# Geo3DSmart/PDANet

Measured on AMD Instinct MI355X. Metric: scenes/sec (16384-pt ONCE, PDA-SSD forward+backward), higher is better.
Workload: dtype f32; 1 GPU; once16k_b2_detector_fwd_bwd_adam; scenes_per_gpu=2, global_batch=2, parallelism=dp1, world_size_seen=1, cpu_affinity=GPU-local NUMA node of 0000:5d:00.0: 128 CPUs, full=False, graph_tail=False, graph_head=True

## Files before the change

### include/pda_train.h

```cpp
#ifndef PDA_TRAIN_H
#define PDA_TRAIN_H
#include "pda_pointnet2.h"

#ifdef __cplusplus
extern "C" {
#endif

int pda_grad_norm(const float *g, int64_t n, float *norm_out, float *scratch1024, pda_stream_t stream);
int pda_adam_onecycle_step(float *p, const float *g, float *m, float *v, int64_t n, float lr,
                           float beta1, float beta2, float eps, float wd, int step,
                           const float *total_norm, float max_norm, pda_stream_t stream);

int64_t pda_bn_relu_scratch_bytes(int c);
int pda_bn_relu_fwd(const float *x, const float *gamma, const float *beta, float *running_mean,
                    float *running_var, float *y, float *mean_invstd, void *scratch, int64_t rows, int c,
                    float eps, float momentum, pda_stream_t stream);
int pda_bn_relu_bwd(const float *x, const float *grad_y, const float *gamma, const float *beta,
                    const float *mean_invstd, float *grad_x, float *grad_gamma, float *grad_beta,
                    void *scratch, int64_t rows, int c, pda_stream_t stream);
int pda_bn_relu_fwd_counted(const float *x, const float *gamma, const float *beta, float *running_mean, float *running_var,
                            float *y, float *mean_invstd, void *scratch, int64_t rows, int c, float eps, float momentum,
                            const int32_t *count, int32_t *status, int relu, int training, pda_stream_t stream);
int pda_bn_relu_bwd_counted(const float *x, const float *grad_y, const float *gamma, const float *beta,
                            const float *mean_invstd, float *grad_x, float *grad_gamma, float *grad_beta, void *scratch,
                            int64_t rows, int c, const int32_t *count, int relu, int training, pda_stream_t stream);
int pda_bn_relu_bwd_reduce(const float *x, const float *grad_y, const float *gamma, const float *beta,
                           const float *mean_invstd, float *grad_gamma, float *grad_beta, float *sums, void *scratch,
                           int64_t rows, int c, pda_stream_t stream);
int pda_bn_relu_fwd_mixed(const void *x, int x_is_bf16, const float *gamma, const float *beta, float *running_mean,
                          float *running_var, void *y, int y_is_bf16, float *mean_invstd, void *scratch,
                          int64_t rows, int c, float eps, float momentum, pda_stream_t stream);
int pda_bn_relu_bwd_mixed(const void *x, int x_is_bf16, const void *grad_y, int grad_y_is_bf16, const float *gamma,
                          const float *beta, const float *mean_invstd, void *grad_x, float *grad_gamma,
                          float *grad_beta, void *scratch, int64_t rows, int c, pda_stream_t stream);
int pda_bn_relu_max_pool_fwd(const void *x, int x_is_bf16, const float *gamma, const float *beta, float *running_mean,
                             float *running_var, float *out, uint8_t *arg, float *mean_invstd, void *scratch,
                             int64_t groups, int ns, int c, float eps, float momentum, pda_stream_t stream);
int pda_bn_relu_max_pool_bwd(const void *x, int x_is_bf16, const float *grad_out, const uint8_t *arg,
                             const float *gamma, const float *beta, const float *mean_invstd, void *grad_x,
                             float *grad_gamma, float *grad_beta, void *scratch, int64_t groups, int ns, int c,
                             pda_stream_t stream);

int64_t pda_layer_norm_scratch_bytes(int d);
int pda_layer_norm_fwd(const float *x, const float *residual, const float *gamma, const float *beta,
                       float *sum_out, float *y, float *mean_rstd, int64_t rows, int d, float eps,
                       pda_stream_t stream);
int pda_layer_norm_bwd(const float *x, const float *grad_y, const float *grad_y2, const float *gamma,
                       const float *mean_rstd, float *grad_x, float *grad_gamma, float *grad_beta,
                       void *scratch, int64_t rows, int d, pda_stream_t stream);
int pda_layer_norm_fwd_mixed(const void *x, int x_is_bf16, const float *residual, const float *gamma,
                             const float *beta, float *sum_out, float *y, uint16_t *y_bf16, float *mean_rstd,
                             int64_t rows, int d, float eps, pda_stream_t stream);
int pda_layer_norm_bwd_mixed(const float *x, const float *grad_y, const void *grad_y2, int grad_y2_is_bf16,
                             const float *gamma, const float *mean_rstd, float *grad_x, uint16_t *grad_x_bf16,
                             float *grad_gamma, float *grad_beta, void *scratch, int64_t rows, int d,
                             pda_stream_t stream);

int64_t pda_linear_wgrad_scratch_bytes(int64_t tokens, int in_features, int out_features);
int pda_linear_wgrad_form(int64_t tokens, int in_features, int out_features);
int pda_linear_wgrad(const float *x, const float *grad_out, float *grad_weight, float *grad_bias,
                     void *scratch, int64_t tokens, int in_features, int out_features, pda_stream_t stream);
int pda_linear_wgrad_bn(const float *x, const float *grad_out, float *grad_weight, float *grad_bias, void *scratch,
                        int64_t tokens, int in_features, int out_features, const float *x_mean_invstd,
                        const float *x_gamma, const float *x_beta, pda_stream_t stream);

int64_t pda_gemm_split_bn_tiles(int64_t tokens);
int pda_gemm_split_bn(const float *x, const void *wf, float *y, int64_t tokens, int k, int n_out,
                      const float *in_mean_invstd, const float *in_gamma, const float *in_beta, int stats_mode,
                      double *partial, pda_stream_t stream);
int pda_gemm_split_maxpool(const float *x, const void *wf, const float *bias, float *out, int64_t tokens, int k, int n_out,
                           int ns, int relu, pda_stream_t stream);
int pda_gemm_split_gather(const float *point_rows, const float *xyz, const float *new_xyz, const int32_t *idx,
                          const float *w1, int ldw1, const float *bias1, const void *wf, const float *bias2, float *y,
                          int b, int n, int m, int ns, int k, int n_out, int relu, pda_stream_t stream);
int pda_bn_stats_fwd(const float *x, float *running_mean, float *running_var, float *mean_invstd, void *scratch,
                     int64_t rows, int c, float eps, float momentum, pda_stream_t stream);
int pda_bn_finalize_fwd(const double *partial, int nblocks, int c, int64_t count, float eps, float momentum,
                        float *mean_invstd, float *running_mean, float *running_var, pda_stream_t stream);
int pda_bn_relu_max_pool_apply(const float *x, const float *gamma, const float *beta, const float *mean_invstd,
                               float *out, uint8_t *arg, int64_t groups, int ns, int c, pda_stream_t stream);

int64_t pda_colsum_scratch_bytes(int cols);
int pda_colsum_bf16(const uint16_t *g, float *out, void *scratch, int64_t rows, int cols, pda_stream_t stream);

int pda_assemble_tokens(const float *rppe, const float *dscale, const float *feats, const int32_t *idx,
                        const float *glob, float *out, int b, int n, int m, int nsample, int c,
                        pda_stream_t stream);
int pda_assemble_tokens_grad(const float *grad_out, const float *dscale, const float *feats, const int32_t *idx,
                             float *grad_rppe, float *grad_dscale, float *grad_feats, float *grad_glob,
                             int b, int n, int m, int nsample, int c, pda_stream_t stream);

int pda_add_max_pool(const float *a, const float *b, float *out, uint8_t *arg, int64_t groups, int seq, int d,
                     pda_stream_t stream);
int pda_max_pool_scatter(const float *grad_out, const uint8_t *arg, float *grad_x, int64_t groups, int seq,
                         int d, pda_stream_t stream);
int pda_add_max_pool_bf16(const float *a, const uint16_t *b, float *out, uint8_t *arg, int64_t groups, int seq,
                          int d, pda_stream_t stream);
int pda_max_pool_scatter_bf16(const float *grad_out, const uint8_t *arg, float *grad_x, uint16_t *grad_x_bf16,
                              int64_t groups, int seq, int d, pda_stream_t stream);

int pda_bn_relu_fwd_weighted(const float *x, const float *gamma, const float *beta, float *running_mean,
                             float *running_var, float *y, float *mean_invstd, void *scratch, int64_t rows, int c,
                             float eps, float momentum, const float *row_weight, int64_t count, pda_stream_t stream);
int pda_bn_relu_bwd_weighted(const float *x, const float *grad_y, const float *gamma, const float *beta,
                             const float *mean_invstd, float *grad_x, float *grad_gamma, float *grad_beta,
                             void *scratch, int64_t rows, int c, const float *row_weight, int64_t count,
                             pda_stream_t stream);

int pda_ragged_plan(const int32_t *idx, int32_t *cnt, int32_t *off, int32_t *rowmap, float *row_weight, int64_t groups,
                    int nsample, pda_stream_t stream);
int pda_assemble_tokens_ragged(const float *rppe, const float *dscale, const float *feats, const int32_t *idx,
                               const float *glob, const int32_t *rowmap, const int32_t *off, float *out,
                               int64_t max_tokens, int b, int n, int m, int nsample, int c, int rppe_compact,
                               pda_stream_t stream);
int pda_assemble_tokens_ragged_grad(const float *grad_out, const float *dscale, const float *feats,
                                    const int32_t *idx, const int32_t *cnt, const int32_t *off, const int32_t *rowmap,
                                    float *grad_rppe, float *grad_dscale, float *grad_feats, float *grad_glob,
                                    int64_t max_tokens, int b, int n, int m, int nsample, int c, int rppe_compact,
                                    pda_stream_t stream);
int pda_add_max_pool_ragged(const float *a, const float *b, const int32_t *cnt, const int32_t *off, float *out,
                            uint8_t *arg, int64_t groups, int d, pda_stream_t stream);
int pda_max_pool_scatter_ragged(const float *grad_out, const uint8_t *arg, const int32_t *rowmap,
                                const int32_t *off, float *grad_x, int64_t max_tokens, int64_t groups, int nsample,
                                int d, pda_stream_t stream);
int pda_group_attention_ragged_fwd(const float *qkv, const int32_t *cnt, const int32_t *off, float *out, float *lse,
                                   int64_t tokens, int64_t num_groups, int seq, int heads, int head_dim,
                                   pda_stream_t stream);
int pda_group_attention_ragged_bwd(const float *qkv, const float *grad_out, const float *lse, const int32_t *cnt,
                                   const int32_t *off, float *grad_qkv, int64_t tokens, int64_t num_groups, int seq,
                                   int heads, int head_dim, pda_stream_t stream);

int pda_densitynet_param_count(void);
int64_t pda_densitynet_scratch_bytes(void);
int pda_densitynet_fwd(const float *x, const float *params, float *y, float *stats, void *scratch,
                       float *running_mean1, float *running_var1, float *running_mean2, float *running_var2,
                       float *running_mean3, float *running_var3, int64_t n, float eps, float momentum,
                       pda_stream_t stream);
int pda_densitynet_bwd(const float *x, const float *grad_y, const float *params, const float *stats,
                       float *grad_params, void *scratch, int64_t n, float eps, pda_stream_t stream);
int pda_densitynet_fwd_unique(const float *x, const float *params, float *y, float *stats, void *scratch,
                              float *running_mean1, float *running_var1, float *running_mean2, float *running_var2,
                              float *running_mean3, float *running_var3, int64_t n, const int32_t *rowmap,
                              const float *row_weight, const int32_t *n_unique, int nsample, float eps, float momentum,
                              pda_stream_t stream);
int pda_densitynet_bwd_unique(const float *x, const float *grad_y, const float *params, const float *stats,
                              float *grad_params, void *scratch, int64_t n, const int32_t *rowmap,
                              const float *row_weight, const int32_t *n_unique, int nsample, float eps,
// ... 390 lines not shown
```

### pdanet_amd/_lib.py

```python
import ctypes
import os

_HERE = os.path.dirname(os.path.abspath(__file__))
LIB_PATH = os.environ.get("PDA_LIB_PATH") or os.path.join(_HERE, "libpda_pointnet2.so")
ABI_VERSION = 20


class DensityNetScale(ctypes.Structure):
    _fields_ = [("x", ctypes.c_void_p), ("grad_y", ctypes.c_void_p), ("params", ctypes.c_void_p), ("y", ctypes.c_void_p),
                ("stats", ctypes.c_void_p), ("scratch", ctypes.c_void_p), ("running", ctypes.c_void_p * 6),
                ("grad_params", ctypes.c_void_p), ("n", ctypes.c_int64), ("rowmap", ctypes.c_void_p),
                ("row_weight", ctypes.c_void_p), ("n_unique", ctypes.c_void_p), ("nsample", ctypes.c_int),
                ("eps", ctypes.c_float), ("momentum", ctypes.c_float)]


class OnceFrames(ctypes.Structure):
    _fields_ = [("gt_boxes", ctypes.c_void_p), ("gt_name", ctypes.c_void_p), ("gt_offsets", ctypes.c_void_p),
                ("pred_boxes", ctypes.c_void_p), ("pred_score", ctypes.c_void_p), ("pred_name", ctypes.c_void_p),
                ("pred_start", ctypes.c_void_p), ("pred_count", ctypes.c_void_p), ("iou_start", ctypes.c_void_p),
                ("n_gt_total", ctypes.c_int64), ("pred_cap", ctypes.c_int64), ("iou_cap", ctypes.c_int64),
                ("n_frames", ctypes.c_int), ("max_gt", ctypes.c_int), ("max_pred", ctypes.c_int)]


class KittiFrames(ctypes.Structure):
    _fields_ = [(n, ctypes.c_void_p) for n in ("gt_bbox", "gt_loc", "gt_dims", "gt_ry", "gt_alpha", "gt_trunc", "gt_occ",
                                               "gt_name", "gt_offsets", "dt_bbox", "dt_box", "dt_alpha", "dt_score",
                                               "dt_name", "dt_start", "dt_count", "ov_start", "frame_mode")] + \
               [("n_gt_total", ctypes.c_int64), ("det_cap", ctypes.c_int64), ("ov_cap", ctypes.c_int64),
                ("n_frames", ctypes.c_int), ("max_gt", ctypes.c_int), ("max_det", ctypes.c_int)]


PARAM_EPOCH = [0]
WEIGHT_EPOCH = [0]

_vp = ctypes.c_void_p
_i = ctypes.c_int
_f = ctypes.c_float

SIGNATURES = {
    "pda_furthest_point_sampling": [_vp, _vp, _vp, _i, _i, _i, _vp],
    "pda_furthest_point_sampling_with_dist": [_vp, _vp, _vp, _i, _i, _i, _vp],
    "pda_gather_points": [_vp, _vp, _vp, _i, _i, _i, _i, _vp],
    "pda_gather_points_grad": [_vp, _vp, _vp, _i, _i, _i, _i, _vp],
    "pda_ball_query": [_vp, _vp, _vp, _i, _i, _i, _f, _i, _vp],
    "pda_ball_query_dilated": [_vp, _vp, _vp, _i, _i, _i, _f, _f, _i, _vp],
    "pda_ellipsoid_query": [_vp, _vp, _vp, _i, _i, _i, _f, _f, _f, _i, _vp],
    "pda_ball_query_cells_scratch_bytes": [_i, _i],
    "pda_ball_query_cells": [_vp, _vp, ctypes.POINTER(_vp), _i, _i, _i, _i, ctypes.POINTER(_f), ctypes.POINTER(ctypes.c_int32),
                             _vp, ctypes.c_int64, _vp],
    "pda_ball_query_multi": [_vp, _vp, ctypes.POINTER(_vp), _i, _i, _i, _i,
                             ctypes.POINTER(_f), ctypes.POINTER(ctypes.c_int32), _vp],
    "pda_group_points": [_vp, _vp, _vp, _i, _i, _i, _i, _i, _vp],
    "pda_group_points_grad": [_vp, _vp, _vp, _i, _i, _i, _i, _i, _vp],
    "pda_group_rows": [_vp, _vp, _vp, _i, _i, _i, ctypes.c_int64, _vp],
    "pda_group_rows_grad": [_vp, _vp, _vp, _i, _i, _i, ctypes.c_int64, _vp],
    "pda_three_nn": [_vp, _vp, _vp, _vp, _i, _i, _i, _vp],
    "pda_three_interpolate": [_vp, _vp, _vp, _vp, _i, _i, _i, _i, _vp],
    "pda_three_interpolate_grad": [_vp, _vp, _vp, _vp, _i, _i, _i, _i, _vp],
    "pda_chamfer_forward": [_vp, _vp, _vp, _vp, _vp, _vp, _i, _i, _i, _vp],
    "pda_chamfer_backward": [_vp, _vp, _vp, _vp, _vp, _vp, _vp, _vp, _i, _i, _i, _vp],
    "pda_group_attention_fwd": [_vp, _vp, _vp, ctypes.c_int64, _i, _i, _i, _vp],
    "pda_group_attention_bwd": [_vp, _vp, _vp, _vp, ctypes.c_int64, _i, _i, _i, _vp],
    "pda_group_attention_fwd_bf16": [_vp, _vp, _vp, ctypes.c_int64, _i, _i, _i, _vp],
    "pda_group_attention_bwd_bf16": [_vp, _vp, _vp, _vp, ctypes.c_int64, _i, _i, _i, _vp],
    "pda_sa_mlp_maxpool": [_vp, _vp, _vp, _vp, _vp, _i, _i, _i, _i, _i, ctypes.POINTER(ctypes.c_int32),
                           ctypes.POINTER(_vp), ctypes.POINTER(_vp), ctypes.POINTER(_vp), _vp],
    "pda_linear_cols_packed_size": [_i, _i],
    "pda_linear_cols_pack": [_vp, _vp, _i, _i, _i, _i, _vp],
    "pda_linear_cols": [_vp, _vp, _vp, ctypes.c_int64, _i, _i, _vp],
    "pda_sa_gather_linear": [_vp, _vp, _vp, _vp, _vp, _vp, _i, _i, _i, _i, _i, _i, _vp],
    "pda_linear_split_packed_bytes": [_i, _i],
    "pda_linear_split_pack": [_vp, _vp, _i, _i, _i, _vp],
    "pda_linear_split_pack_both": [_vp, _vp, _vp, _i, _i, _vp],
    "pda_linear_split": [_vp, _vp, _vp, _vp, ctypes.c_int64, _i, _i, _i, _vp],
    "pda_gemm_split": [_vp, _vp, _vp, _vp, ctypes.c_int64, _i, _i, _i, _i, _vp],
    "pda_sa_mlp_packed_size": [_i, _i, _i],
    "pda_sa_mlp_pack_weights": [_vp, _vp, _i, _i, _i, _vp],
    "pda_grad_norm": [_vp, ctypes.c_int64, _vp, _vp, _vp],
    "pda_bn_relu_scratch_bytes": [_i],
    "pda_bn_relu_fwd": [_vp, _vp, _vp, _vp, _vp, _vp, _vp, _vp, ctypes.c_int64, _i, _f, _f, _vp],
    "pda_bn_relu_bwd": [_vp, _vp, _vp, _vp, _vp, _vp, _vp, _vp, _vp, ctypes.c_int64, _i, _vp],    "pda_bn_relu_fwd_mixed": [_vp, _i, _vp, _vp, _vp, _vp, _vp, _i, _vp, _vp, ctypes.c_int64, _i, _f, _f, _vp],
    "pda_bn_relu_bwd_mixed": [_vp, _i, _vp, _i, _vp, _vp, _vp, _vp, _vp, _vp, _vp, ctypes.c_int64, _i, _vp],
    "pda_bn_relu_max_pool_fwd": [_vp, _i, _vp, _vp, _vp, _vp, _vp, _vp, _vp, _vp, ctypes.c_int64, _i, _i, _f, _f, _vp],
    "pda_bn_relu_max_pool_bwd": [_vp, _i, _vp, _vp, _vp, _vp, _vp, _vp, _vp, _vp, _vp, ctypes.c_int64, _i, _i, _vp],

    "pda_layer_norm_scratch_bytes": [_i],
    "pda_layer_norm_fwd": [_vp, _vp, _vp, _vp, _vp, _vp, _vp, ctypes.c_int64, _i, _f, _vp],
    "pda_layer_norm_bwd": [_vp, _vp, _vp, _vp, _vp, _vp, _vp, _vp, _vp, ctypes.c_int64, _i, _vp],
    "pda_layer_norm_fwd_mixed": [_vp, _i, _vp, _vp, _vp, _vp, _vp, _vp, _vp, ctypes.c_int64, _i, _f, _vp],
    "pda_layer_norm_bwd_mixed": [_vp, _vp, _vp, _i, _vp, _vp, _vp, _vp, _vp, _vp, _vp, ctypes.c_int64, _i, _vp],
    "pda_linear_wgrad_scratch_bytes": [ctypes.c_int64, _i, _i],
    "pda_linear_wgrad_form": [ctypes.c_int64, _i, _i],
    "pda_linear_wgrad": [_vp, _vp, _vp, _vp, _vp, ctypes.c_int64, _i, _i, _vp],
    "pda_linear_wgrad_bn": [_vp, _vp, _vp, _vp, _vp, ctypes.c_int64, _i, _i, _vp, _vp, _vp, _vp],
    "pda_gemm_split_bn_tiles": [ctypes.c_int64],
    "pda_gemm_split_bn": [_vp, _vp, _vp, ctypes.c_int64, _i, _i, _vp, _vp, _vp, _i, _vp, _vp],
    "pda_gemm_split_maxpool": [_vp, _vp, _vp, _vp, ctypes.c_int64, _i, _i, _i, _i, _vp],
    "pda_gemm_split_gather": [_vp, _vp, _vp, _vp, _vp, _i, _vp, _vp, _vp, _vp, _i, _i, _i, _i, _i, _i, _i, _vp],
    "pda_bn_stats_fwd": [_vp, _vp, _vp, _vp, _vp, ctypes.c_int64, _i, _f, _f, _vp],
    "pda_bn_finalize_fwd": [_vp, _i, _i, ctypes.c_int64, _f, _f, _vp, _vp, _vp, _vp],
    "pda_bn_relu_max_pool_apply": [_vp, _vp, _vp, _vp, _vp, _vp, ctypes.c_int64, _i, _i, _vp],
    "pda_bn_relu_bwd_reduce": [_vp, _vp, _vp, _vp, _vp, _vp, _vp, _vp, _vp, ctypes.c_int64, _i, _vp],
    "pda_colsum_scratch_bytes": [_i],
    "pda_colsum_bf16": [_vp, _vp, _vp, ctypes.c_int64, _i, _vp],
    "pda_assemble_tokens": [_vp, _vp, _vp, _vp, _vp, _vp, _i, _i, _i, _i, _i, _vp],
    "pda_assemble_tokens_grad": [_vp, _vp, _vp, _vp, _vp, _vp, _vp, _vp, _i, _i, _i, _i, _i, _vp],
    "pda_add_max_pool": [_vp, _vp, _vp, _vp, ctypes.c_int64, _i, _i, _vp],
    "pda_max_pool_scatter": [_vp, _vp, _vp, ctypes.c_int64, _i, _i, _vp],
    "pda_add_max_pool_bf16": [_vp, _vp, _vp, _vp, ctypes.c_int64, _i, _i, _vp],
    "pda_max_pool_scatter_bf16": [_vp, _vp, _vp, _vp, ctypes.c_int64, _i, _i, _vp],
    "pda_ragged_plan": [_vp, _vp, _vp, _vp, _vp, ctypes.c_int64, _i, _vp],
    "pda_assemble_tokens_ragged": [_vp, _vp, _vp, _vp, _vp, _vp, _vp, _vp, ctypes.c_int64, _i, _i, _i, _i, _i, _i, _vp],
    "pda_assemble_tokens_ragged_grad": [_vp, _vp, _vp, _vp, _vp, _vp, _vp, _vp, _vp, _vp, _vp, ctypes.c_int64, _i, _i, _i, _i, _i, _i, _vp],
    "pda_bn_relu_fwd_weighted": [_vp, _vp, _vp, _vp, _vp, _vp, _vp, _vp, ctypes.c_int64, _i, _f, _f, _vp, ctypes.c_int64, _vp],
    "pda_bn_relu_bwd_weighted": [_vp, _vp, _vp, _vp, _vp, _vp, _vp, _vp, _vp, ctypes.c_int64, _i, _vp, ctypes.c_int64, _vp],
    "pda_add_max_pool_ragged": [_vp, _vp, _vp, _vp, _vp, _vp, ctypes.c_int64, _i, _vp],
    "pda_max_pool_scatter_ragged": [_vp, _vp, _vp, _vp, _vp, ctypes.c_int64, ctypes.c_int64, _i, _i, _vp],
    "pda_group_attention_ragged_fwd": [_vp, _vp, _vp, _vp, _vp, ctypes.c_int64, ctypes.c_int64, _i, _i, _i, _vp],
    "pda_group_attention_ragged_bwd": [_vp, _vp, _vp, _vp, _vp, _vp, ctypes.c_int64, ctypes.c_int64, _i, _i, _i, _vp],
    "pda_densitynet_param_count": [],
    "pda_densitynet_eval_param_count": [],
    "pda_densitynet_scratch_bytes": [],
    "pda_densitynet_fwd": [_vp, _vp, _vp, _vp, _vp, _vp, _vp, _vp, _vp, _vp, _vp, ctypes.c_int64, _f, _f, _vp],
    "pda_densitynet_bwd": [_vp, _vp, _vp, _vp, _vp, _vp, ctypes.c_int64, _f, _vp],
    "pda_densitynet_eval": [_vp, _vp, _vp, ctypes.c_int64, _vp],
    "pda_densitynet_fwd_multi": [_vp, _i, _vp],
    "pda_densitynet_bwd_multi": [_vp, _i, _vp],
    "pda_densitynet_fwd_unique": [_vp, _vp, _vp, _vp, _vp, _vp, _vp, _vp, _vp, _vp, _vp, ctypes.c_int64, _vp, _vp, _vp, _i, _f, _f, _vp],
    "pda_densitynet_bwd_unique": [_vp, _vp, _vp, _vp, _vp, _vp, ctypes.c_int64, _vp, _vp, _vp, _i, _f, _vp],
    "pda_pda_geometry": [_vp, _vp, _vp, _vp, _vp, _i, _i, _i, _i, _f, _vp],
    "pda_points_in_boxes": [_vp, _vp, _vp, _i, _i, _i, _vp],
    "pda_roiaware_pool3d_fwd": [_vp, _vp, _vp, _vp, _vp, _vp, _i, _i, _i, _i, _i, _i, _i, _i, _vp],
    "pda_roiaware_pool3d_bwd": [_vp, _vp, _vp, _vp, _i, _i, _i, _i, _i, _i, _i, _i, _vp],
    "pda_roipoint_pool3d_fwd": [_vp, _vp, _vp, _vp, _vp, _i, _i, _i, _i, _i, _vp],
    "pda_points_in_boxes_mask": [_vp, _vp, _vp, _i, _i, _vp],
    "pda_points_in_boxes_count": [_vp, _i, _vp, _vp, _i, _i, _i, _vp],
    "pda_assign_point_targets": [_vp, _vp, _vp, _vp, _vp, _vp, _i, _i, _i, _i, _i, _vp],
    "pda_sa_gaussian_mask": [_vp, _i, _i, _vp, _vp, _vp, ctypes.c_int64, _vp],
    "pda_head_assign_targets": [_vp, _i, _i, _vp, ctypes.POINTER(ctypes.c_float), _vp, _vp, _vp, _vp, _vp, _i, _i, _i, _i, _i, _i, _vp],
    "pda_head_cls_loss": [_vp, _i, _i, _i, _vp, _vp, ctypes.c_int64, _f, _vp, _vp, _vp],
    "pda_head_centerness": [_vp, _vp, _vp, _vp, ctypes.c_int64, _vp],
    "pda_head_box_loss": [_vp, _vp, _vp, _vp, _f, _i, _f, _f, ctypes.c_int64, _vp, _vp, _vp],
    "pda_head_vote_loss": [_i, _vp, _vp, _vp, _vp, _i, _i, _i, _f, ctypes.c_int64, _vp, _vp, _vp],
    "pda_head_corner_loss": [_vp, _vp, _vp, _i, _vp, _vp, _vp, _i, _f, ctypes.c_int64, _vp, _vp, _vp, _vp],
    "pda_boxes_overlap_bev": [_vp, _vp, _vp, _i, _i, _vp],
    "pda_boxes_iou_bev": [_vp, _vp, _vp, _i, _i, _vp],
    "pda_nms_mask_words": [_i],
    "pda_nms_bev": [_vp, _vp, _vp, _vp, _vp, _i, _i, _f, _i, _vp],
    "pda_sa_small_train_workspace_bytes": [],
    "pda_sa_small_train_supported": [_i, _i, _i, _i, _i, ctypes.c_int64],
    "pda_sa_small_train_fwd": [_vp] * 7 + [ctypes.POINTER(_vp)] * 4 + [ctypes.POINTER(_f)] * 2 + [_vp] * 4 + [_i] * 8 + [_vp],
    "pda_sa_small_train_bwd": [_vp] * 13 + [ctypes.POINTER(_vp)] * 2 + [_i] * 8 + [_vp],
    "pda_sa_xyz_grad_scratch_bytes": [_i],
    "pda_sa_point_gather": [_vp, _vp, _vp, _vp, _vp, _i, _vp, _i, _vp, _i, _i, _i, _i, _i, _vp],
    "pda_sa_xyz_grad": [_vp, _vp, _vp, _vp, _vp, _i, _vp, _i, _vp, _vp, _i, _i, _i, _i, _i, _vp],
    "pda_sa_point_gather_stats_blocks": [ctypes.c_int64, _i],
    "pda_sa_point_gather_stats": [_vp, _vp, _vp, _vp, _vp, _i, _vp, _vp, _i, _i, _i, _i, _i, _vp],
    "pda_sa_point_grad_bn": [_vp] * 10 + [_i, _vp, _i, _vp, _vp, _vp, _i, _i, _i, _i, _i, _vp],
    "pda_adam_onecycle_step": [_vp, _vp, _vp, _vp, ctypes.c_int64, _f, _f, _f, _f, _f, _i, _vp, _f, _vp],
    "pda_input_stage_workspace_bytes": [_i, ctypes.c_int64],
    "pda_input_stage": [_vp, _vp, ctypes.c_int64, _i, _i, ctypes.c_int64, ctypes.POINTER(_f), _i, _vp, _vp, _vp,
                        ctypes.c_uint64, _i, _vp, _vp, _vp, _vp],
    "pda_input_boxes": [_vp, _vp, ctypes.c_int64, _i, _i, _i, ctypes.POINTER(_f), _i, _vp, _vp, _vp],
    "pda_augment_workspace_bytes": [_i, ctypes.c_int64, _i],
    "pda_augment": [_vp, _vp, ctypes.c_int64, _i, _i, ctypes.c_int64, _vp, _vp, ctypes.c_int64, _vp, _vp, ctypes.c_int64, _vp,
                    _vp, _vp, _i, _vp, _vp, _vp, _i, _vp, _vp, _vp, ctypes.POINTER(_f), ctypes.c_int64, _vp, ctypes.c_int64,
                    _vp, _vp, ctypes.c_int64, _vp, _vp, _vp, _vp],
    "pda_augment_paste": [_vp, _vp, ctypes.c_int64, _i, _i, ctypes.c_int64, _vp, _vp, ctypes.c_int64, _vp, _vp, ctypes.c_int64, _vp,
                          _vp, _vp, _i, _vp, _vp, _vp, _i, ctypes.POINTER(_f), ctypes.c_int64, _vp, ctypes.c_int64, _vp, _vp,
                          ctypes.c_int64, _vp, _vp, _vp, _vp],
    "pda_augment_steps_workspace_bytes": [_i, ctypes.c_int64, _i, _i],
    "pda_augment_steps": [_vp, _vp, ctypes.c_int64, _i, _i, ctypes.c_int64, _vp, _vp, ctypes.c_int64,
                          ctypes.POINTER(ctypes.c_int32), _i, _vp, _vp, _i, _i, _vp, _vp, ctypes.c_int64, _vp, _vp,
                          ctypes.c_int64, _vp, _vp, _vp, _vp],
    "pda_pyramid_aug_workspace_bytes": [_i, ctypes.c_int64, _i],
    "pda_pyramid_aug": [_vp, _vp, ctypes.c_int64, _i, _i, ctypes.c_int64, _vp, _vp, ctypes.c_int64, _vp, _vp, _vp, _vp, _vp, _i,
                        ctypes.POINTER(ctypes.c_double), _i, _i, _i, _vp, _vp, ctypes.c_int64, _vp, _vp, ctypes.c_int64, _vp,
# ... 172 lines not shown
```

### pdanet_amd/csrc/layer_norm.hip

```cpp
#include "pda_common.h"

namespace pda {

constexpr int LN_BLOCKS = 1024;

__device__ __forceinline__ float wave_sum(float v) {
#pragma unroll
    for (int o = 32; o >= 1; o >>= 1) v += __shfl_xor(v, o);
    return v;
}

template <int V, bool RESIDUAL, typename TX>
__global__ __launch_bounds__(256) void layer_norm_fwd_kernel(const TX* __restrict__ x, const float* __restrict__ res,
                                                             const float* __restrict__ gamma, const float* __restrict__ beta,
                                                             float* __restrict__ sum_out, float* __restrict__ y,
                                                             bf16_t* __restrict__ yb, float* __restrict__ mean_rstd, int64_t rows,
                                                             float eps) {
    constexpr int D = 256 * V;
    const int lane = lane_id();
    float4 g[V], be[V];
#pragma unroll
    for (int v = 0; v < V; ++v) {
        g[v] = reinterpret_cast<const float4*>(gamma)[v * 64 + lane];
        be[v] = reinterpret_cast<const float4*>(beta)[v * 64 + lane];
    }
    for (int64_t r = (int64_t)blockIdx.x * 4 + wave_id(); r < rows; r += (int64_t)gridDim.x * 4) {
        float4 a[V];
        float s = 0.f;
#pragma unroll
        for (int v = 0; v < V; ++v) {
            a[v] = load4(x + r * D + 4 * (v * 64 + lane));
            if (RESIDUAL) {
                const float4 b = reinterpret_cast<const float4*>(res + r * D)[v * 64 + lane];
                a[v].x += b.x; a[v].y += b.y; a[v].z += b.z; a[v].w += b.w;
                reinterpret_cast<float4*>(sum_out + r * D)[v * 64 + lane] = a[v];
            }
            s += (a[v].x + a[v].y) + (a[v].z + a[v].w);
        }
        const float mean = wave_sum(s) * (1.0f / D);
        float q = 0.f;
#pragma unroll
        for (int v = 0; v < V; ++v) {
            const float dx = a[v].x - mean, dy = a[v].y - mean, dz = a[v].z - mean, dw = a[v].w - mean;
            q += (dx * dx + dy * dy) + (dz * dz + dw * dw);
        }
        const float rstd = 1.0f / sqrtf(wave_sum(q) * (1.0f / D) + eps);
#pragma unroll
        for (int v = 0; v < V; ++v) {
            float4 o;
            o.x = (a[v].x - mean) * rstd * g[v].x + be[v].x;
            o.y = (a[v].y - mean) * rstd * g[v].y + be[v].y;
            o.z = (a[v].z - mean) * rstd * g[v].z + be[v].z;
            o.w = (a[v].w - mean) * rstd * g[v].w + be[v].w;
            if (y) reinterpret_cast<float4*>(y + r * D)[v * 64 + lane] = o;
            if (yb) store4(yb + r * D + 4 * (v * 64 + lane), o);
        }
        if (lane == 0) { mean_rstd[r * 2] = mean; mean_rstd[r * 2 + 1] = rstd; }
    }
}

template <int V, bool TWO, typename T2>
__global__ __launch_bounds__(256) void layer_norm_bwd_kernel(const float* __restrict__ x, const float* __restrict__ dy,
                                                             const T2* __restrict__ dy2, const float* __restrict__ gamma,
                                                             const float* __restrict__ mean_rstd, float* __restrict__ dx,
                                                             bf16_t* __restrict__ dxb, float* __restrict__ partial, int64_t rows) {
    constexpr int D = 256 * V;
    __shared__ float red[2][4][D];
    const int lane = lane_id(), w = wave_id();
    float4 g[V], sb[V], sg[V];
#pragma unroll
    for (int v = 0; v < V; ++v) {
        g[v] = reinterpret_cast<const float4*>(gamma)[v * 64 + lane];
        sb[v] = make_float4(0, 0, 0, 0); sg[v] = make_float4(0, 0, 0, 0);
    }
    for (int64_t r = (int64_t)blockIdx.x * 4 + w; r < rows; r += (int64_t)gridDim.x * 4) {
        const float mean = mean_rstd[r * 2], rstd = mean_rstd[r * 2 + 1];
        float4 xh[V], d[V];
        float s1 = 0.f, s2 = 0.f;
#pragma unroll
        for (int v = 0; v < V; ++v) {
            const float4 xv = reinterpret_cast<const float4*>(x + r * D)[v * 64 + lane];
            d[v] = reinterpret_cast<const float4*>(dy + r * D)[v * 64 + lane];
            if (TWO) {
                const float4 e = load4(dy2 + r * D + 4 * (v * 64 + lane));
                d[v].x += e.x; d[v].y += e.y; d[v].z += e.z; d[v].w += e.w;
            }
            xh[v] = make_float4((xv.x - mean) * rstd, (xv.y - mean) * rstd, (xv.z - mean) * rstd, (xv.w - mean) * rstd);
            sb[v].x += d[v].x; sb[v].y += d[v].y; sb[v].z += d[v].z; sb[v].w += d[v].w;
            sg[v].x += d[v].x * xh[v].x; sg[v].y += d[v].y * xh[v].y; sg[v].z += d[v].z * xh[v].z; sg[v].w += d[v].w * xh[v].w;
            d[v].x *= g[v].x; d[v].y *= g[v].y; d[v].z *= g[v].z; d[v].w *= g[v].w;
            s1 += (d[v].x + d[v].y) + (d[v].z + d[v].w);
            s2 += (d[v].x * xh[v].x + d[v].y * xh[v].y) + (d[v].z * xh[v].z + d[v].w * xh[v].w);
        }
        const float m1 = wave_sum(s1) * (1.0f / D), m2 = wave_sum(s2) * (1.0f / D);
#pragma unroll
        for (int v = 0; v < V; ++v) {
            float4 o;
            o.x = rstd * (d[v].x - m1 - xh[v].x * m2);
            o.y = rstd * (d[v].y - m1 - xh[v].y * m2);
            o.z = rstd * (d[v].z - m1 - xh[v].z * m2);
            o.w = rstd * (d[v].w - m1 - xh[v].w * m2);
            reinterpret_cast<float4*>(dx + r * D)[v * 64 + lane] = o;
            if (dxb) store4(dxb + r * D + 4 * (v * 64 + lane), o);
        }
    }
#pragma unroll
    for (int v = 0; v < V; ++v) {
        reinterpret_cast<float4*>(red[0][w])[v * 64 + lane] = sb[v];
        reinterpret_cast<float4*>(red[1][w])[v * 64 + lane] = sg[v];
    }
    __syncthreads();
    for (int c = threadIdx.x; c < D; c += 256) {
        partial[((size_t)blockIdx.x * 2 + 0) * D + c] = (red[0][0][c] + red[0][1][c]) + (red[0][2][c] + red[0][3][c]);
        partial[((size_t)blockIdx.x * 2 + 1) * D + c] = (red[1][0][c] + red[1][1][c]) + (red[1][2][c] + red[1][3][c]);
    }
}

__global__ __launch_bounds__(1024) void layer_norm_finalize_kernel(const float* __restrict__ partial, int nblocks, int d,
                                                                   float* __restrict__ dgamma, float* __restrict__ dbeta) {
    __shared__ float red[2][16][64];
    const int cl = threadIdx.x & 63, part = threadIdx.x >> 6;
    const int c = blockIdx.x * 64 + cl;
    float a = 0.f, b = 0.f;
    if (c < d) {
        float va[8], vb[8];
        for (int k0 = part; k0 < nblocks; k0 += 16 * 8) {
#pragma unroll
            for (int u = 0; u < 8; ++u) {
                const int k = k0 + 16 * u;
                va[u] = k < nblocks ? partial[((size_t)k * 2 + 0) * d + c] : 0.f;
                vb[u] = k < nblocks ? partial[((size_t)k * 2 + 1) * d + c] : 0.f;
            }
#pragma unroll
            for (int u = 0; u < 8; ++u) { a += va[u]; b += vb[u]; }
        }
    }
    red[0][part][cl] = a; red[1][part][cl] = b;
    __syncthreads();
    if (part != 0 || c >= d) return;
    float s1 = 0.f, s2 = 0.f;
#pragma unroll
    for (int p = 0; p < 16; ++p) { s1 += red[0][p][cl]; s2 += red[1][p][cl]; }
    dbeta[c] = s1;
    dgamma[c] = s2;
}

static int ln_grid(int64_t rows) {
    const int64_t b = divup64(rows, 4);
    return (int)(b < LN_BLOCKS ? b : LN_BLOCKS);
}

}

PDA_API int64_t pda_layer_norm_scratch_bytes(int d) { return (int64_t)pda::LN_BLOCKS * 2 * (d > 0 ? d : 0) * (int64_t)sizeof(float); }

namespace pda {

template <typename TX>
static int launch_layer_norm_fwd(const TX* x, const float* residual, const float* gamma, const float* beta, float* sum_out, float* y,
                                 bf16_t* yb, float* mean_rstd, int64_t rows, int d, float eps, hipStream_t st, const char* what) {
    PDA_REQUIRE(rows >= 0, "%s: rows = %lld", what, (long long)rows);
    PDA_REQUIRE(d == 256 || d == 512 || d == 1024, "%s: D = %d (256, 512 or 1024)", what, d);
    if (rows == 0) return PDA_OK;
    PDA_REQUIRE(x && gamma && beta && (y || yb) && mean_rstd, "%s: null pointer", what);
    PDA_REQUIRE((residual == nullptr) == (sum_out == nullptr), "%s: residual and sum_out come together", what);
    PDA_REQUIRE((((uintptr_t)y | (uintptr_t)gamma | (uintptr_t)beta | (uintptr_t)residual | (uintptr_t)sum_out) & 15) == 0 &&
                    (((uintptr_t)x | (uintptr_t)yb) & (4 * sizeof(TX) - 1) & 15) == 0 && ((uintptr_t)yb & 7) == 0,
                "%s: pointers must be 16-byte aligned (8 for bf16 tensors)", what);
    const dim3 grid(ln_grid(rows)), block(256);
#define PDA_LN_FWD(V)                                                                                                          \
    if (residual) hipLaunchKernelGGL((layer_norm_fwd_kernel<V, true, TX>), grid, block, 0, st, x, residual, gamma, beta, sum_out, y, yb, mean_rstd, rows, eps); \
    else hipLaunchKernelGGL((layer_norm_fwd_kernel<V, false, TX>), grid, block, 0, st, x, residual, gamma, beta, sum_out, y, yb, mean_rstd, rows, eps)
    if (d == 256) { PDA_LN_FWD(1); } else if (d == 512) { PDA_LN_FWD(2); } else { PDA_LN_FWD(4); }
#undef PDA_LN_FWD
    return check_launch(what);
}

template <typename T2>
static int launch_layer_norm_bwd(const float* x, const float* grad_y, const T2* grad_y2, const float* gamma, const float* mean_rstd,
                                 float* grad_x, bf16_t* grad_x_b, float* grad_gamma, float* grad_beta, void* scratch, int64_t rows, int d,
                                 hipStream_t st, const char* what) {
    PDA_REQUIRE(rows >= 1, "%s: rows = %lld", what, (long long)rows);
    PDA_REQUIRE(d == 256 || d == 512 || d == 1024, "%s: D = %d (256, 512 or 1024)", what, d);
    PDA_REQUIRE(x && grad_y && gamma && mean_rstd && grad_x && grad_gamma && grad_beta && scratch, "%s: null pointer", what);
    PDA_REQUIRE((((uintptr_t)x | (uintptr_t)grad_y | (uintptr_t)grad_x | (uintptr_t)gamma) & 15) == 0 &&
                    ((uintptr_t)grad_y2 & (4 * sizeof(T2) - 1)) == 0 && ((uintptr_t)grad_x_b & 7) == 0,
                "%s: pointers must be 16-byte aligned (8 for bf16 tensors)", what);
    const int nblocks = ln_grid(rows);
    const dim3 grid(nblocks), block(256);
    float* partial = (float*)scratch;
#define PDA_LN_BWD(V)                                                                                                               \
    if (grad_y2) hipLaunchKernelGGL((layer_norm_bwd_kernel<V, true, T2>), grid, block, 0, st, x, grad_y, grad_y2, gamma, mean_rstd, grad_x, grad_x_b, partial, rows); \
    else hipLaunchKernelGGL((layer_norm_bwd_kernel<V, false, T2>), grid, block, 0, st, x, grad_y, grad_y2, gamma, mean_rstd, grad_x, grad_x_b, partial, rows)
    if (d == 256) { PDA_LN_BWD(1); } else if (d == 512) { PDA_LN_BWD(2); } else { PDA_LN_BWD(4); }
#undef PDA_LN_BWD
    hipLaunchKernelGGL(layer_norm_finalize_kernel, dim3(divup(d, 64)), dim3(1024), 0, st, partial, nblocks, d, grad_gamma, grad_beta);
    return check_launch(what);
}

}

PDA_API int pda_layer_norm_fwd(const float* x, const float* residual, const float* gamma, const float* beta, float* sum_out,
                               float* y, float* mean_rstd, int64_t rows, int d, float eps, pda_stream_t stream) {
    PDA_REQUIRE(y != nullptr || rows == 0, "pda_layer_norm_fwd: null pointer");
    return pda::launch_layer_norm_fwd<float>(x, residual, gamma, beta, sum_out, y, nullptr, mean_rstd, rows, d, eps, (hipStream_t)stream,
                                             "pda_layer_norm_fwd");
}

PDA_API int pda_layer_norm_fwd_mixed(const void* x, int x_is_bf16, const float* residual, const float* gamma, const float* beta,
                                     float* sum_out, float* y, uint16_t* y_bf16, float* mean_rstd, int64_t rows, int d, float eps,
                                     pda_stream_t stream) {
    if (x_is_bf16)
        return pda::launch_layer_norm_fwd<pda::bf16_t>((const pda::bf16_t*)x, residual, gamma, beta, sum_out, y, y_bf16, mean_rstd, rows, d,
                                                       eps, (hipStream_t)stream, "pda_layer_norm_fwd_mixed");
    return pda::launch_layer_norm_fwd<float>((const float*)x, residual, gamma, beta, sum_out, y, y_bf16, mean_rstd, rows, d, eps,
                                             (hipStream_t)stream, "pda_layer_norm_fwd_mixed");
}

PDA_API int pda_layer_norm_bwd(const float* x, const float* grad_y, const float* grad_y2, const float* gamma, const float* mean_rstd,
                               float* grad_x, float* grad_gamma, float* grad_beta, void* scratch, int64_t rows, int d,
                               pda_stream_t stream) {
    return pda::launch_layer_norm_bwd<float>(x, grad_y, grad_y2, gamma, mean_rstd, grad_x, nullptr, grad_gamma, grad_beta, scratch, rows, d,
                                             (hipStream_t)stream, "pda_layer_norm_bwd");
}

PDA_API int pda_layer_norm_bwd_mixed(const float* x, const float* grad_y, const void* grad_y2, int grad_y2_is_bf16, const float* gamma,
                                     const float* mean_rstd, float* grad_x, uint16_t* grad_x_bf16, float* grad_gamma, float* grad_beta,
                                     void* scratch, int64_t rows, int d, pda_stream_t stream) {
    if (grad_y2_is_bf16)
        return pda::launch_layer_norm_bwd<pda::bf16_t>(x, grad_y, (const pda::bf16_t*)grad_y2, gamma, mean_rstd, grad_x, grad_x_bf16,
                                                       grad_gamma, grad_beta, scratch, rows, d, (hipStream_t)stream, "pda_layer_norm_bwd_mixed");
    return pda::launch_layer_norm_bwd<float>(x, grad_y, (const float*)grad_y2, gamma, mean_rstd, grad_x, grad_x_bf16, grad_gamma, grad_beta,
                                             scratch, rows, d, (hipStream_t)stream, "pda_layer_norm_bwd_mixed");
}

namespace pda {

template <typename TB>
__global__ __launch_bounds__(256) void add_max_pool_kernel(const float* __restrict__ a, const TB* __restrict__ b,
                                                           float* __restrict__ out, uint8_t* __restrict__ arg, int64_t groups,
                                                           int s, int d4) {
    const int64_t e = (int64_t)blockIdx.x * 256 + threadIdx.x;
    if (e >= groups * d4) return;
    const int64_t g = e / d4;
    const int c = (int)(e % d4);
    const float4* pa = reinterpret_cast<const float4*>(a) + (size_t)g * s * d4 + c;
    const TB* pb = b + 4 * ((size_t)g * s * d4 + c);
    float4 best = make_float4(-__builtin_inff(), -__builtin_inff(), -__builtin_inff(), -__builtin_inff());
    uchar4 bi = make_uchar4(0, 0, 0, 0);
    for (int t = 0; t < s; ++t) {
        const float4 x = pa[(size_t)t * d4], y = load4(pb + 4 * (size_t)t * d4);
        const float4 v = make_float4(x.x + y.x, x.y + y.y, x.z + y.z, x.w + y.w);
        if (v.x > best.x) { best.x = v.x; bi.x = (uint8_t)t; }
        if (v.y > best.y) { best.y = v.y; bi.y = (uint8_t)t; }
        if (v.z > best.z) { best.z = v.z; bi.z = (uint8_t)t; }
        if (v.w > best.w) { best.w = v.w; bi.w = (uint8_t)t; }
    }
    reinterpret_cast<float4*>(out)[e] = best;
    reinterpret_cast<uchar4*>(arg)[e] = bi;
}

__global__ __launch_bounds__(256) void max_pool_scatter_kernel(const float* __restrict__ dout, const uint8_t* __restrict__ arg,
                                                               float* __restrict__ dx, bf16_t* __restrict__ dxb, int64_t groups, int s,
                                                               int d4) {
    const int64_t e = (int64_t)blockIdx.x * 256 + threadIdx.x;
    if (e >= groups * s * d4) return;
    const int c = (int)(e % d4);
    const int t = (int)((e / d4) % s);
    const int64_t g = e / ((int64_t)d4 * s);
    const float4 v = reinterpret_cast<const float4*>(dout)[g * d4 + c];
    const uchar4 k = reinterpret_cast<const uchar4*>(arg)[g * d4 + c];
    const float4 o = make_float4(k.x == t ? v.x : 0.f, k.y == t ? v.y : 0.f, k.z == t ? v.z : 0.f, k.w == t ? v.w : 0.f);
    reinterpret_cast<float4*>(dx)[e] = o;
    if (dxb) store4(dxb + 4 * e, o);
}

}

namespace pda {

template <typename TB>
static int launch_add_max_pool(const float* a, const TB* b, float* out, uint8_t* arg, int64_t groups, int seq, int d, hipStream_t st,
                               const char* what) {
    PDA_REQUIRE(groups >= 0 && seq >= 1 && seq <= 255 && d >= 4 && (d & 3) == 0, "%s: groups=%lld seq=%d d=%d", what, (long long)groups, seq, d);
    if (groups == 0) return PDA_OK;
    PDA_REQUIRE(a && b && out && arg, "%s: null pointer", what);
    PDA_REQUIRE((((uintptr_t)a | (uintptr_t)out) & 15) == 0 && ((uintptr_t)b & (4 * sizeof(TB) - 1)) == 0 && ((uintptr_t)arg & 3) == 0,
                "%s: alignment", what);
    const int64_t n = groups * (d / 4);
    hipLaunchKernelGGL(add_max_pool_kernel<TB>, dim3((unsigned)divup64(n, 256)), dim3(256), 0, st, a, b, out, arg, groups, seq, d / 4);
    return check_launch(what);
}

static int launch_max_pool_scatter(const float* grad_out, const uint8_t* arg, float* grad_x, bf16_t* grad_x_b, int64_t groups, int seq, int d,
                                   hipStream_t st, const char* what) {
    PDA_REQUIRE(groups >= 0 && seq >= 1 && seq <= 255 && d >= 4 && (d & 3) == 0, "%s: groups=%lld seq=%d d=%d", what, (long long)groups, seq, d);
    if (groups == 0) return PDA_OK;
    PDA_REQUIRE(grad_out && arg && grad_x, "%s: null pointer", what);
    PDA_REQUIRE((((uintptr_t)grad_out | (uintptr_t)grad_x) & 15) == 0 && ((uintptr_t)arg & 3) == 0 && ((uintptr_t)grad_x_b & 7) == 0,
                "%s: alignment", what);
    const int64_t n = groups * seq * (d / 4);
    hipLaunchKernelGGL(max_pool_scatter_kernel, dim3((unsigned)divup64(n, 256)), dim3(256), 0, st, grad_out, arg, grad_x, grad_x_b, groups,
                       seq, d / 4);
    return check_launch(what);
}

}

PDA_API int pda_add_max_pool(const float* a, const float* b, float* out, uint8_t* arg, int64_t groups, int seq, int d,
                             pda_stream_t stream) {
    return pda::launch_add_max_pool<float>(a, b, out, arg, groups, seq, d, (hipStream_t)stream, "pda_add_max_pool");
}

PDA_API int pda_add_max_pool_bf16(const float* a, const uint16_t* b, float* out, uint8_t* arg, int64_t groups, int seq, int d,
                                  pda_stream_t stream) {
    return pda::launch_add_max_pool<pda::bf16_t>(a, b, out, arg, groups, seq, d, (hipStream_t)stream, "pda_add_max_pool_bf16");
// ... 13 lines not shown
```

### pdanet_amd/csrc/wgrad.hip

```cpp
#include "pda_common.h"
#include "split_bf16.h"

#include <stdlib.h>

namespace pda {

typedef float f32x16 __attribute__((ext_vector_type(16)));

constexpr int WG_KC = 32;
constexpr int WG_TILE = 128;

__device__ __forceinline__ void lds_dma16(const float* gsrc, float* lds_dst_wave_uniform) {
    uint32_t keep;
    const uint32_t dst = __builtin_amdgcn_readfirstlane((uint32_t)(uintptr_t)lds_dst_wave_uniform);
    asm volatile("s_mov_b32 %0, m0\n\ts_mov_b32 m0, %2\n\ts_nop 0\n\tglobal_load_lds_dwordx4 %1, off\n\ts_mov_b32 m0, %0"
                 : "=&s"(keep) : "v"(gsrc), "s"(dst) : "memory");
}

__global__ __launch_bounds__(256) void wgrad_kernel(const float* __restrict__ X, const float* __restrict__ G,
                                                    float* __restrict__ part_w, float* __restrict__ part_b, int64_t T, int M,
                                                    int N, int tiles_m, int tiles_n, int S, int64_t KS, int nblocks) {
    __shared__ __attribute__((aligned(16))) float ldsG[2][WG_KC][WG_TILE];
    __shared__ __attribute__((aligned(16))) float ldsX[2][WG_KC][WG_TILE];
    const int per_xcd = (nblocks + 7) / 8;
    const int logical = (int)(blockIdx.x & 7) * per_xcd + (int)(blockIdx.x >> 3);
    if (logical >= nblocks) return;
    const int tiles = tiles_m * tiles_n;
    const int tile = logical % tiles, s = logical / tiles;
    const int n0 = (tile / tiles_m) * WG_TILE, m0 = (tile % tiles_m) * WG_TILE;
    const int64_t t_begin = (int64_t)s * KS, t_end = (t_begin + KS < T) ? t_begin + KS : T;

    const int tid = threadIdx.x, lane = lane_id(), w = wave_id();
    const int c = lane & 31, h = lane >> 5;
    const int wn = w >> 1, wm = w & 1;
    const int lrow = tid >> 5, lcol = (tid & 31) * 4;
    const bool g_ok = n0 + lcol < N, x_ok = m0 + lcol < M;

    f32x16 acc[2][2];
#pragma unroll
    for (int i = 0; i < 2; ++i)
#pragma unroll
        for (int j = 0; j < 2; ++j)
#pragma unroll
            for (int r = 0; r < 16; ++r) acc[i][j][r] = 0.f;
    float bsum[2] = {0.f, 0.f};

    float4 rg[4], rx[4];
    const int gcol = g_ok ? n0 + lcol : 0, xcol = x_ok ? m0 + lcol : 0;
    auto load_chunk = [&](int64_t t0) {
#pragma unroll
        for (int p = 0; p < 4; ++p) {
            const int64_t t = t0 + p * 8 + lrow;
            const bool in = t < t_end;
            const int64_t tc = in ? t : t_end - 1;
            const float4 vg = *reinterpret_cast<const float4*>(G + tc * N + gcol);
            const float4 vx = *reinterpret_cast<const float4*>(X + tc * M + xcol);
            rg[p] = (in && g_ok) ? vg : make_float4(0.f, 0.f, 0.f, 0.f);
            rx[p] = (in && x_ok) ? vx : make_float4(0.f, 0.f, 0.f, 0.f);
        }
    };
    auto store_chunk = [&](int buf) {
#pragma unroll
        for (int p = 0; p < 4; ++p) {
            *reinterpret_cast<float4*>(&ldsG[buf][p * 8 + lrow][lcol]) = rg[p];
            *reinterpret_cast<float4*>(&ldsX[buf][p * 8 + lrow][lcol]) = rx[p];
        }
    };

    const bool full_tile = (n0 + WG_TILE <= N) && (m0 + WG_TILE <= M);
    auto dma_chunk = [&](int64_t t0, int b) {
#pragma unroll
        for (int i = 0; i < 4; ++i) {
            const int row = w * 8 + 2 * i;
            const int64_t t = t0 + row + (lane >> 5);
            const int col = (lane & 31) * 4;
            lds_dma16(G + t * N + n0 + col, &ldsG[b][row][0]);
            lds_dma16(X + t * M + m0 + col, &ldsX[b][row][0]);
        }
    };
    auto compute = [&](int buf) {
        float fa[2][2], fb[2][2];
        fa[0][0] = ldsG[buf][h][wn * 64 + c]; fa[0][1] = ldsG[buf][h][wn * 64 + 32 + c];
        fb[0][0] = ldsX[buf][h][wm * 64 + c]; fb[0][1] = ldsX[buf][h][wm * 64 + 32 + c];
#pragma unroll
// ... 166 lines not shown
        out[0] = make_uint4(ph[0], ph[1], ph[2], ph[3]);
        out[64] = make_uint4(pm[0], pm[1], pm[2], pm[3]);
        out[128] = make_uint4(pl[0], pl[1], pl[2], pl[3]);
        bsum += ((ga[0] + ga[1]) + (ga[2] + ga[3])) + ((ga[4] + ga[5]) + (ga[6] + ga[7]));
        read_b(2);
#pragma unroll
        for (int q = 0; q < 4; ++q) {
            mfma3(An, 1, q);
            __builtin_amdgcn_sched_barrier(0);
#if WSP_ABL == 1
            ph[q] = __float_as_uint(xa[2 * q]); pm[q] = __float_as_uint(xa[2 * q + 1]); pl[q] = ph[q] ^ pm[q];
#else
            split2(xt(xa[2 * q]), xt(xa[2 * q + 1]), ph[q], pm[q], pl[q]);
#endif
            __builtin_amdgcn_sched_barrier(0);
        }
        out[8 * 192] = make_uint4(ph[0], ph[1], ph[2], ph[3]);
        out[8 * 192 + 64] = make_uint4(pm[0], pm[1], pm[2], pm[3]);
        out[8 * 192 + 128] = make_uint4(pl[0], pl[1], pl[2], pl[3]);
        read_b(3);
#pragma unroll
        for (int q = 0; q < 4; ++q) {
            mfma3(An, 2, q);
#if WSP_ABL != 3
            __builtin_amdgcn_sched_barrier(0);
            load1(st + 2, 2 * q, gb, xb);
            load1(st + 2, 2 * q + 1, gb, xb);
            __builtin_amdgcn_sched_barrier(0);
#endif
        }
    };
    auto split_store = [&](const float (&g)[8], const float (&x)[8], int b) {
        uint4* out = my_planes + b * WSP_TILE_U4;
        uint32_t ph[4], pm[4], pl[4];
#pragma unroll
        for (int q = 0; q < 4; ++q) split2(g[2 * q], g[2 * q + 1], ph[q], pm[q], pl[q]);
        out[0] = make_uint4(ph[0], ph[1], ph[2], ph[3]);
        out[64] = make_uint4(pm[0], pm[1], pm[2], pm[3]);
        out[128] = make_uint4(pl[0], pl[1], pl[2], pl[3]);
#pragma unroll
        for (int q = 0; q < 4; ++q) split2(xt(x[2 * q]), xt(x[2 * q + 1]), ph[q], pm[q], pl[q]);
        out[8 * 192] = make_uint4(ph[0], ph[1], ph[2], ph[3]);
        out[8 * 192 + 64] = make_uint4(pm[0], pm[1], pm[2], pm[3]);
        out[8 * 192 + 128] = make_uint4(pl[0], pl[1], pl[2], pl[3]);
        bsum += ((g[0] + g[1]) + (g[2] + g[3])) + ((g[4] + g[5]) + (g[6] + g[7]));
    };
    float g1[8], x1[8], g2[8], x2[8];
    gs_bf16x8 A0[2][3], A1[2][3];
#pragma unroll
    for (int i = 0; i < 2; ++i)
#pragma unroll
        for (int pl = 0; pl < 3; ++pl) {
            A0[i][pl] = __builtin_bit_cast(gs_bf16x8, make_uint4(0u, 0u, 0u, 0u));
            Bf[1][pl] = A0[i][pl];
        }
    load(0, g1, x1);
    split_store(g1, x1, 0);
    load(1, g1, x1);
    for (int st = 0; st < ksteps; st += 2) {
        step(st, g1, x1, g2, x2, A0, A1);
        step(st + 1, g2, x2, g1, x1, A1, A0);
    }
#pragma unroll
    for (int e = 0; e < 12; ++e)
        acc[e & 1][3] = __builtin_amdgcn_mfma_f32_32x32x16_bf16(A0[e & 1][PA[e >> 1]], Bf[1][PB[e >> 1]], acc[e & 1][3], 0, 0, 0);
    float* pw = part_w + (size_t)s * N * M;
#pragma unroll
    for (int i = 0; i < 2; ++i)
#pragma unroll
        for (int jt = 0; jt < 4; ++jt) {
            const int m = m0 + 128 * wm + 32 * jt + c;
#pragma unroll
            for (int r = 0; r < 16; ++r) {
                const int n = n0 + 64 * wn + 32 * i + (r & 3) + 8 * (r >> 2) + 4 * h;
                pw[(size_t)n * M + m] = acc[i][jt][r];
            }
        }
    if (do_bias) {
        const float v = bsum + __shfl_xor(bsum, 32);
        if (h == 0) part_b[(size_t)s * N + n0 + 32 * w + c] = v;
    }
}

__device__ __forceinline__ float sum_slices(const float* __restrict__ part, int S, int64_t stride, int64_t e, bool live, int slice,
                                            float (*red)[64], int el) {
    float a = 0.f;
    if (live) {
        float v[8];
        for (int s0 = slice; s0 < S; s0 += 16 * 8) {
#pragma unroll
            for (int u = 0; u < 8; ++u) {
                const int sidx = s0 + 16 * u;
                v[u] = sidx < S ? part[(size_t)sidx * stride + e] : 0.f;
            }
#pragma unroll
            for (int u = 0; u < 8; ++u) a += v[u];
        }
    }
    red[slice][el] = a;
    __syncthreads();
    float r = 0.f;
    if (slice == 0)
#pragma unroll
        for (int p = 0; p < 16; ++p) r += red[p][el];
    __syncthreads();
    return r;
}

__global__ __launch_bounds__(1024) void wgrad_reduce_kernel(const float* __restrict__ part_w, const float* __restrict__ part_b,
                                                            float* __restrict__ dw, float* __restrict__ db, int S, int64_t nm, int N) {
    __shared__ float red[16][64];
    const int el = threadIdx.x & 63, slice = threadIdx.x >> 6;
    const int64_t e = (int64_t)blockIdx.x * 64 + el;
    const float w = sum_slices(part_w, S, nm, e, e < nm, slice, red, el);
    if (slice == 0 && e < nm) dw[e] = w;
    if (db && (int64_t)blockIdx.x * 64 < N) {
        const float bsum = sum_slices(part_b, S, N, e, e < N, slice, red, el);
        if (slice == 0 && e < N) db[e] = bsum;
    }
}

constexpr int WS_UNROLL = 8;
constexpr int WS_MAX_SLICES = 1024;

template <int NT, int MT>
__global__ __launch_bounds__(256) void wgrad_skinny_kernel(const float* __restrict__ X, const float* __restrict__ G,
                                                           float* __restrict__ part_w, float* __restrict__ part_b, int64_t T, int M,
                                                           int N, int64_t KS) {
    __shared__ float red[NT * MT * 1024 + 64 * NT];
    const int tid = threadIdx.x, lane = lane_id(), w = wave_id();
    const int i = lane & 31, h = lane >> 5;
    const int64_t t_begin = (int64_t)blockIdx.x * KS, t_end = (t_begin + KS < T) ? t_begin + KS : T;
    f32x16 acc[NT][MT];
    float sb[NT];
#pragma unroll
    for (int a = 0; a < NT; ++a) {
        sb[a] = 0.f;
#pragma unroll
        for (int b = 0; b < MT; ++b)
#pragma unroll
            for (int r = 0; r < 16; ++r) acc[a][b][r] = 0.f;
    }
    bool gcol[NT], xcol[MT];
#pragma unroll
    for (int a = 0; a < NT; ++a) gcol[a] = a * 32 + i < N;
#pragma unroll
    for (int b = 0; b < MT; ++b) xcol[b] = b * 32 + i < M;
    for (int64_t t0 = t_begin + 2 * w; t0 < t_end; t0 += 8 * WS_UNROLL) {
        float ga[WS_UNROLL][NT], xb[WS_UNROLL][MT];
#pragma unroll
        for (int u = 0; u < WS_UNROLL; ++u) {
            const int64_t t = t0 + 8 * u + h;
            const bool ok = t < t_end;
#pragma unroll
            for (int a = 0; a < NT; ++a) ga[u][a] = (ok && gcol[a]) ? G[t * N + a * 32 + i] : 0.f;
#pragma unroll
            for (int b = 0; b < MT; ++b) xb[u][b] = (ok && xcol[b]) ? X[t * M + b * 32 + i] : 0.f;
        }
#pragma unroll
        for (int u = 0; u < WS_UNROLL; ++u)
#pragma unroll
            for (int a = 0; a < NT; ++a) {
                sb[a] += ga[u][a];
#pragma unroll
                for (int b = 0; b < MT; ++b) acc[a][b] = __builtin_amdgcn_mfma_f32_32x32x2f32(ga[u][a], xb[u][b], acc[a][b], 0, 0, 0);
            }
    }
    for (int turn = 0; turn < 4; ++turn) {
        if (w == turn) {
#pragma unroll
            for (int a = 0; a < NT; ++a) {
#pragma unroll
                for (int b = 0; b < MT; ++b)
#pragma unroll
                    for (int r = 0; r < 16; ++r) {
                        float* d = red + ((a * MT + b) * 32 + (r & 3) + 8 * (r >> 2) + 4 * h) * 32 + i;
                        *d = turn == 0 ? acc[a][b][r] : *d + acc[a][b][r];
                    }
                float* d = red + NT * MT * 1024 + a * 64 + lane;
                *d = turn == 0 ? sb[a] : *d + sb[a];
            }
        }
        __syncthreads();
    }
    float* pw = part_w + (size_t)blockIdx.x * N * M;
    for (int e = tid; e < NT * MT * 1024; e += 256) {
        const int tile = e >> 10, n = (tile / MT) * 32 + ((e >> 5) & 31), m = (tile % MT) * 32 + (e & 31);
        if (n < N && m < M) pw[n * M + m] = red[e];
    }
    if (part_b) {
        for (int n = tid; n < N; n += 256) {
            const int o = NT * MT * 1024 + (n >> 5) * 64 + (n & 31);
            part_b[(size_t)blockIdx.x * N + n] = red[o] + red[o + 32];
        }
    }
}

static bool wgrad_is_skinny(int M, int N) { return M <= 64 && N <= 64; }
static void wgrad_skinny_plan(int64_t T, int& S, int64_t& KS) {
    int64_t s = T / 512 > 0 ? T / 512 : 1;
    if (s > WS_MAX_SLICES) s = WS_MAX_SLICES;
    KS = divup64(divup64(T, s), 8) * 8;
    S = (int)divup64(T, KS);
}

static void wgrad_plan(int64_t T, int M, int N, int& tiles_m, int& tiles_n, int& S, int64_t& KS) {
    tiles_m = divup(M, WG_TILE); tiles_n = divup(N, WG_TILE);
    const int tiles = tiles_m * tiles_n;
    int64_t s = 512 / tiles;
    if (T / s < 128 && tiles <= 256) s = 256 / tiles;
    const int64_t max_s = T / 64 > 0 ? T / 64 : 1;
    if (s > max_s) s = max_s;
    if (s < 1) s = 1;
    KS = divup64(divup64(T, s), WG_KC) * WG_KC;
    S = (int)divup64(T, KS);
}

static bool wgrad_use_split(int64_t T, int M, int N) {
    static const int mode = [] { const char* e = getenv("PDA_WGRAD_SPLIT"); return e ? atoi(e) : 1; }();
    if (mode == 0 || (M & 255) || (N & 255) || T < 4096) return false;
    return mode == 2 || (double)T * M * N >= 2.0e9;
}
static void wgrad_split_plan(int64_t T, int M, int N, int& tiles_m, int& tiles_n, int& S, int64_t& KS) {
    tiles_m = M / 256; tiles_n = N / 256;
    const int tiles = tiles_m * tiles_n;
    int64_t s = 256 / tiles;
    const int64_t max_s = T / 256 > 0 ? T / 256 : 1;
    if (s > max_s) s = max_s;
    const int64_t min_s = divup64(T * (M > N ? M : N) * 4, (int64_t)1 << 31);
    if (s < min_s) s = min_s;
    if (s < 1) s = 1;
    KS = divup64(divup64(T, s), 16) * 16;
    S = (int)divup64(T, KS);
}

}

PDA_API int64_t pda_linear_wgrad_scratch_bytes(int64_t tokens, int in_features, int out_features) {
    if (tokens <= 0 || in_features <= 0 || out_features <= 0) return 0;
    int tm, tn, S;
    int64_t KS;
    if (pda::wgrad_is_skinny(in_features, out_features)) pda::wgrad_skinny_plan(tokens, S, KS);
    else if (pda::wgrad_use_split(tokens, in_features, out_features)) pda::wgrad_split_plan(tokens, in_features, out_features, tm, tn, S, KS);
    else pda::wgrad_plan(tokens, in_features, out_features, tm, tn, S, KS);
    return (int64_t)S * ((int64_t)in_features * out_features + out_features) * (int64_t)sizeof(float);
}

PDA_API int pda_linear_wgrad_form(int64_t tokens, int in_features, int out_features) {
    if (pda::wgrad_is_skinny(in_features, out_features)) return 1;
    return pda::wgrad_use_split(tokens, in_features, out_features) ? 2 : 0;
}

namespace pda {
static int linear_wgrad(const float* x, const float* grad_out, float* grad_weight, float* grad_bias, void* scratch, int64_t tokens,
                        int in_features, int out_features, pda_stream_t stream, const float* x_mi, const float* x_g, const float* x_b);
}

PDA_API int pda_linear_wgrad(const float* x, const float* grad_out, float* grad_weight, float* grad_bias, void* scratch,
                             int64_t tokens, int in_features, int out_features, pda_stream_t stream) {
    return pda::linear_wgrad(x, grad_out, grad_weight, grad_bias, scratch, tokens, in_features, out_features, stream, nullptr, nullptr, nullptr);
}

PDA_API int pda_linear_wgrad_bn(const float* x, const float* grad_out, float* grad_weight, float* grad_bias, void* scratch,
                                int64_t tokens, int in_features, int out_features, const float* x_mean_invstd, const float* x_gamma,
                                const float* x_beta, pda_stream_t stream) {
    PDA_REQUIRE(x_mean_invstd && x_gamma && x_beta, "pda_linear_wgrad_bn: null pointer");
    if (pda_linear_wgrad_form(tokens, in_features, out_features) != 2) {
        pda::set_error("pda_linear_wgrad_bn: tokens=%lld in=%d out=%d does not run on the split form", (long long)tokens, in_features, out_features);
        return PDA_ERR_UNSUPPORTED;
    }
    return pda::linear_wgrad(x, grad_out, grad_weight, grad_bias, scratch, tokens, in_features, out_features, stream, x_mean_invstd, x_gamma, x_beta);
}

int pda::linear_wgrad(const float* x, const float* grad_out, float* grad_weight, float* grad_bias, void* scratch, int64_t tokens,
                             int in_features, int out_features, pda_stream_t stream, const float* x_mi, const float* x_g, const float* x_b) {
    const int M = in_features, N = out_features;
    PDA_REQUIRE(tokens >= 1 && M >= 4 && N >= 4 && (M & 3) == 0 && (N & 3) == 0,
                "pda_linear_wgrad: tokens=%lld in=%d out=%d (features must be multiples of 4)", (long long)tokens, M, N);
    PDA_REQUIRE(x && grad_out && grad_weight && scratch, "pda_linear_wgrad: null pointer");
    PDA_REQUIRE((((uintptr_t)x | (uintptr_t)grad_out) & 15) == 0, "pda_linear_wgrad: x / grad_out must be 16-byte aligned");
    int tm, tn, S;
    int64_t KS;
    hipStream_t st = (hipStream_t)stream;
    if (pda::wgrad_is_skinny(M, N)) {
        pda::wgrad_skinny_plan(tokens, S, KS);
        float* pw = (float*)scratch;
        float* pb = grad_bias ? pw + (size_t)S * N * M : (float*)nullptr;
        const int nt = N > 32 ? 2 : 1, mt = M > 32 ? 2 : 1;
#define PDA_WS_CASE(A, B) hipLaunchKernelGGL((pda::wgrad_skinny_kernel<A, B>), dim3(S), dim3(256), 0, st, x, grad_out, pw, pb, tokens, M, N, KS)
        if (nt == 1 && mt == 1) PDA_WS_CASE(1, 1);
        else if (nt == 1) PDA_WS_CASE(1, 2);
        else if (mt == 1) PDA_WS_CASE(2, 1);
        else PDA_WS_CASE(2, 2);
#undef PDA_WS_CASE
        const int64_t nm = (int64_t)N * M;
        hipLaunchKernelGGL(pda::wgrad_reduce_kernel, dim3((unsigned)pda::divup64(nm, 64)), dim3(1024), 0, st, pw, pb, grad_weight,
                           grad_bias, S, nm, N);
        return pda::check_launch("pda_linear_wgrad");
    }
    if (pda::wgrad_use_split(tokens, M, N)) {
        pda::wgrad_split_plan(tokens, M, N, tm, tn, S, KS);
        const int nblocks = S * tm * tn;
        float* part_w = (float*)scratch;
        float* part_b = part_w + (size_t)S * N * M;
        static pda::PerDevice<bool> lds_ok;
        const bool ok = lds_ok.get([] {
            return hipFuncSetAttribute((const void*)pda::wgrad_split_kernel<false>, hipFuncAttributeMaxDynamicSharedMemorySize, 2 * pda::WSP_TILE_U4 * 16) == hipSuccess &&
                   hipFuncSetAttribute((const void*)pda::wgrad_split_kernel<true>, hipFuncAttributeMaxDynamicSharedMemorySize, 2 * pda::WSP_TILE_U4 * 16) == hipSuccess; });
        PDA_REQUIRE(ok, "pda_linear_wgrad: %d bytes of dynamic LDS refused", 2 * pda::WSP_TILE_U4 * 16);
        if (x_mi)
            hipLaunchKernelGGL(pda::wgrad_split_kernel<true>, dim3(pda::divup(nblocks, 8) * 8), dim3(512), 2 * pda::WSP_TILE_U4 * 16, st,
                               x, grad_out, part_w, grad_bias ? part_b : (float*)nullptr, tokens, M, N, tm, tn, S, KS, nblocks, x_mi, x_g, x_b);
        else
            hipLaunchKernelGGL(pda::wgrad_split_kernel<false>, dim3(pda::divup(nblocks, 8) * 8), dim3(512), 2 * pda::WSP_TILE_U4 * 16, st,
                               x, grad_out, part_w, grad_bias ? part_b : (float*)nullptr, tokens, M, N, tm, tn, S, KS, nblocks, x_mi, x_g, x_b);
        const int64_t nm = (int64_t)N * M;
        hipLaunchKernelGGL(pda::wgrad_reduce_kernel, dim3((unsigned)pda::divup64(nm, 64)), dim3(1024), 0, st, part_w, part_b,
                           grad_weight, grad_bias, S, nm, N);
        return pda::check_launch("pda_linear_wgrad");
    }
    pda::wgrad_plan(tokens, M, N, tm, tn, S, KS);
    const int nblocks = S * tm * tn;
    float* part_w = (float*)scratch;
    float* part_b = part_w + (size_t)S * N * M;
    hipLaunchKernelGGL(pda::wgrad_kernel, dim3(pda::divup(nblocks, 8) * 8), dim3(256), 0, st, x, grad_out, part_w,
                       grad_bias ? part_b : (float*)nullptr, tokens, M, N, tm, tn, S, KS, nblocks);
    const int64_t nm = (int64_t)N * M;
    hipLaunchKernelGGL(pda::wgrad_reduce_kernel, dim3((unsigned)pda::divup64(nm, 64)), dim3(1024), 0, st, part_w, part_b, grad_weight,
                       grad_bias, S, nm, N);
    return pda::check_launch("pda_linear_wgrad");
}

namespace pda {

constexpr int CS_BLOCKS = 512;

__global__ __launch_bounds__(256) void colsum_bf16_kernel(const bf16_t* __restrict__ g, float* __restrict__ partial, int64_t rows,
                                                          int cols, int nv, int rpb) {
    __shared__ float lds[256 * 8];
    const int tid = threadIdx.x;
    float acc[8] = {0.f, 0.f, 0.f, 0.f, 0.f, 0.f, 0.f, 0.f};
    const int v = tid % nv, r0 = tid / nv;
    if (tid < nv * rpb) {
        for (int64_t r = (int64_t)blockIdx.x * rpb + r0; r < rows; r += (int64_t)gridDim.x * rpb) {
            const uint4 u = *reinterpret_cast<const uint4*>(g + r * cols + 8 * v);
            acc[0] += __uint_as_float(u.x << 16); acc[1] += __uint_as_float(u.x & 0xffff0000u);
            acc[2] += __uint_as_float(u.y << 16); acc[3] += __uint_as_float(u.y & 0xffff0000u);
            acc[4] += __uint_as_float(u.z << 16); acc[5] += __uint_as_float(u.z & 0xffff0000u);
            acc[6] += __uint_as_float(u.w << 16); acc[7] += __uint_as_float(u.w & 0xffff0000u);
        }
    }
#pragma unroll
    for (int k = 0; k < 8; ++k) lds[tid * 8 + k] = acc[k];
    __syncthreads();
    if (tid < nv) {
        float s[8] = {0.f, 0.f, 0.f, 0.f, 0.f, 0.f, 0.f, 0.f};
        for (int r = 0; r < rpb; ++r)
#pragma unroll
            for (int k = 0; k < 8; ++k) s[k] += lds[(r * nv + tid) * 8 + k];
#pragma unroll
        for (int k = 0; k < 8; ++k) partial[(size_t)blockIdx.x * cols + 8 * tid + k] = s[k];
    }
}

__global__ __launch_bounds__(256) void colsum_final_kernel(const float* __restrict__ partial, int nblocks, int cols,
                                                           float* __restrict__ out) {
    __shared__ double red[16][16];
    const int cl = threadIdx.x & 15, part = threadIdx.x >> 4;
    const int c = blockIdx.x * 16 + cl;
    double a = 0.0;
    if (c < cols) {
        float va[8];
        for (int k0 = part; k0 < nblocks; k0 += 16 * 8) {
#pragma unroll
            for (int u = 0; u < 8; ++u) {
                const int k = k0 + 16 * u;
                va[u] = k < nblocks ? partial[(size_t)k * cols + c] : 0.f;
            }
#pragma unroll
            for (int u = 0; u < 8; ++u) a += (double)va[u];
        }
    }
    red[part][cl] = a;
    __syncthreads();
    if (part != 0 || c >= cols) return;
    double s = 0.0;
#pragma unroll
    for (int p = 0; p < 16; ++p) s += red[p][cl];
    out[c] = (float)s;
}

}

PDA_API int64_t pda_colsum_scratch_bytes(int cols) { return (int64_t)pda::CS_BLOCKS * (cols > 0 ? cols : 0) * (int64_t)sizeof(float); }

PDA_API int pda_colsum_bf16(const uint16_t* g, float* out, void* scratch, int64_t rows, int cols, pda_stream_t stream) {
    PDA_REQUIRE(rows >= 1 && cols >= 8 && cols <= 2048 && (cols & 7) == 0, "pda_colsum_bf16: rows=%lld cols=%d (cols: multiple of 8, <= 2048)",
                (long long)rows, cols);
    PDA_REQUIRE(g && out && scratch, "pda_colsum_bf16: null pointer");
    PDA_REQUIRE(((uintptr_t)g & 15) == 0, "pda_colsum_bf16: g must be 16-byte aligned");
    const int nv = cols / 8, rpb = 256 / nv;
    const int64_t steps = pda::divup64(rows, (int64_t)rpb * 8);
    const int grid = (int)(steps < pda::CS_BLOCKS ? steps : pda::CS_BLOCKS);
    hipStream_t st = (hipStream_t)stream;
    hipLaunchKernelGGL(pda::colsum_bf16_kernel, dim3(grid), dim3(256), 0, st, g, (float*)scratch, rows, cols, nv, rpb);
    hipLaunchKernelGGL(pda::colsum_final_kernel, dim3(pda::divup(cols, 16)), dim3(256), 0, st, (const float*)scratch, grid, cols, out);
    return pda::check_launch("pda_colsum_bf16");
}
```

### pdanet_amd/pointnet2_batch_cuda.py

```python
import ctypes

import functools

import torch

from . import _lib
from . import param_cache


def _chk(t, name, dtype):
    if not isinstance(t, torch.Tensor):
        raise TypeError("%s must be a torch.Tensor" % name)
    if not t.is_cuda:
        raise RuntimeError("%s must be a CUDA(HIP) tensor -- there is no CPU path" % name)
    if not t.is_contiguous():
        raise RuntimeError("%s must be contiguous" % name)
    if t.dtype != dtype:
        raise RuntimeError("%s must be %s, got %s" % (name, dtype, t.dtype))
    return t.data_ptr()


def _numel_ok(t, n, name):
    if t.numel() < n:
        raise RuntimeError("%s has %d elements, the sizes passed need %d" % (name, t.numel(), n))


def _stream(t):
    return torch._C._cuda_getCurrentRawStream(t.device.index)


_FNS = {}


def _call(fn_name, tensor, *args):
    fn = _FNS.get(fn_name)
    if fn is None:
        fn = _FNS[fn_name] = getattr(_lib.load(), fn_name)
    idx = tensor.device.index
    if idx == torch._C._cuda_getDevice():
        st = fn(*args, torch._C._cuda_getCurrentRawStream(idx))
    else:
        with torch.cuda.device(tensor.device):
            st = fn(*args, torch._C._cuda_getCurrentRawStream(idx))
    if st != 0:
        _lib.check(st, fn_name)


F32, I32 = torch.float32, torch.int32


def _ptr_array(items):
    return (ctypes.c_void_p * len(items))(*[t.data_ptr() if isinstance(t, torch.Tensor) else t for t in items])


def _partials(blocks_fn, n, device):
    return torch.empty((3 * int(getattr(_lib.load(), blocks_fn)(n)),), dtype=torch.float64, device=device)


def ball_query_wrapper(b, n, m, radius, nsample, new_xyz, xyz, idx):
    _numel_ok(new_xyz, b * m * 3, "new_xyz"); _numel_ok(xyz, b * n * 3, "xyz")
    _numel_ok(idx, b * m * nsample, "idx")
    _call("pda_ball_query", xyz, _chk(new_xyz, "new_xyz", F32), _chk(xyz, "xyz", F32),
          _chk(idx, "idx", I32), b, n, m, float(radius), nsample)
    return 1


def ball_query_dilated_wrapper(b, n, m, max_radius, min_radius, nsample, new_xyz, xyz, idx):
    _numel_ok(new_xyz, b * m * 3, "new_xyz"); _numel_ok(xyz, b * n * 3, "xyz")
    _numel_ok(idx, b * m * nsample, "idx")
    _call("pda_ball_query_dilated", xyz, _chk(new_xyz, "new_xyz", F32), _chk(xyz, "xyz", F32),
          _chk(idx, "idx", I32), b, n, m, float(max_radius), float(min_radius), nsample)
    return 1


def fps_coop_timeouts(reset=False):
    total = ctypes.c_ulonglong(0)
    _lib.check(_lib.load().pda_fps_coop_timeouts(ctypes.byref(total), 1 if reset else 0), "pda_fps_coop_timeouts")
    return int(total.value)


def debug_fps_spin_limit(polls):
    _lib.check(_lib.load().pda_debug_fps_spin_limit(int(polls)), "pda_debug_fps_spin_limit")


def ellipsoid_query(new_xyz, xyz, e1, e2, e3, nsample):
# ... 183 lines not shown
    if x.dtype == F32 and y.dtype == F32:
        _call("pda_bn_relu_fwd", x, _chk(x, "x", F32), _chk(gamma, "gamma", F32), _chk(beta, "beta", F32), rm, rv,
              _chk(y, "y", F32), _chk(mean_invstd, "mean_invstd", F32), _chk(scratch, "scratch", torch.uint8), rows, c,
              float(eps), float(momentum))
        return 1
    (xp, xb), (yp, yb) = _io(x, "x"), _io(y, "y")
    _call("pda_bn_relu_fwd_mixed", x, xp, xb, _chk(gamma, "gamma", F32), _chk(beta, "beta", F32), rm, rv, yp, yb,
          _chk(mean_invstd, "mean_invstd", F32), _chk(scratch, "scratch", torch.uint8), rows, c, float(eps), float(momentum))
    return 1


def bn_relu_bwd(x, grad_y, gamma, beta, mean_invstd, grad_x, grad_gamma, grad_beta, scratch, rows, c):
    _numel_ok(x, rows * c, "x"); _numel_ok(grad_y, rows * c, "grad_y"); _numel_ok(grad_x, rows * c, "grad_x")
    if x.dtype == F32 and grad_y.dtype == F32:
        _call("pda_bn_relu_bwd", x, _chk(x, "x", F32), _chk(grad_y, "grad_y", F32), _chk(gamma, "gamma", F32),
              _chk(beta, "beta", F32), _chk(mean_invstd, "mean_invstd", F32), _chk(grad_x, "grad_x", F32),
              _chk(grad_gamma, "grad_gamma", F32), _chk(grad_beta, "grad_beta", F32), _chk(scratch, "scratch", torch.uint8), rows, c)
        return 1
    (xp, xb), (gp, gb) = _io(x, "x"), _io(grad_y, "grad_y")
    _call("pda_bn_relu_bwd_mixed", x, xp, xb, gp, gb, _chk(gamma, "gamma", F32), _chk(beta, "beta", F32),
          _chk(mean_invstd, "mean_invstd", F32), _chk(grad_x, "grad_x", x.dtype), _chk(grad_gamma, "grad_gamma", F32),
          _chk(grad_beta, "grad_beta", F32), _chk(scratch, "scratch", torch.uint8), rows, c)
    return 1


def bn_relu_bwd_reduce(x, grad_y, gamma, beta, mean_invstd, grad_gamma, grad_beta, sums, scratch, rows, c):
    _numel_ok(x, rows * c, "x"); _numel_ok(grad_y, rows * c, "grad_y"); _numel_ok(sums, 2 * c, "sums")
    _numel_ok(grad_gamma, c, "grad_gamma"); _numel_ok(grad_beta, c, "grad_beta"); _numel_ok(mean_invstd, 2 * c, "mean_invstd")
    _call("pda_bn_relu_bwd_reduce", x, _chk(x, "x", F32), _chk(grad_y, "grad_y", F32), _chk(gamma, "gamma", F32), _chk(beta, "beta", F32),
          _chk(mean_invstd, "mean_invstd", F32), _chk(grad_gamma, "grad_gamma", F32), _chk(grad_beta, "grad_beta", F32),
          _chk(sums, "sums", F32), _chk(scratch, "scratch", torch.uint8), rows, c)
    return 1


def bn_relu_max_pool_fwd(x, gamma, beta, running_mean, running_var, out, arg, mean_invstd, scratch, groups, ns, c, eps, momentum):
    _numel_ok(x, groups * ns * c, "x"); _numel_ok(out, groups * c, "out"); _numel_ok(arg, groups * c, "arg"); _numel_ok(mean_invstd, 2 * c, "mean_invstd")
    rm = None if running_mean is None else _chk(running_mean, "running_mean", F32)
    rv = None if running_var is None else _chk(running_var, "running_var", F32)
    _buffers_written(rm)
    xp, xb = _io(x, "x")
    _call("pda_bn_relu_max_pool_fwd", x, xp, xb, _chk(gamma, "gamma", F32), _chk(beta, "beta", F32), rm, rv, _chk(out, "out", F32),
          _chk(arg, "arg", torch.uint8), _chk(mean_invstd, "mean_invstd", F32), _chk(scratch, "scratch", torch.uint8), groups, ns, c,
          float(eps), float(momentum))
    return 1


def bn_relu_max_pool_bwd(x, grad_out, arg, gamma, beta, mean_invstd, grad_x, grad_gamma, grad_beta, scratch, groups, ns, c):
    _numel_ok(x, groups * ns * c, "x"); _numel_ok(grad_out, groups * c, "grad_out"); _numel_ok(arg, groups * c, "arg")
    _numel_ok(grad_x, groups * ns * c, "grad_x")
    xp, xb = _io(x, "x")
    _call("pda_bn_relu_max_pool_bwd", x, xp, xb, _chk(grad_out, "grad_out", F32), _chk(arg, "arg", torch.uint8), _chk(gamma, "gamma", F32),
          _chk(beta, "beta", F32), _chk(mean_invstd, "mean_invstd", F32), _chk(grad_x, "grad_x", x.dtype), _chk(grad_gamma, "grad_gamma", F32),
          _chk(grad_beta, "grad_beta", F32), _chk(scratch, "scratch", torch.uint8), groups, ns, c)
    return 1


@functools.lru_cache(maxsize=None)
def layer_norm_scratch_bytes(d):
    return int(_lib.load().pda_layer_norm_scratch_bytes(int(d)))


BF16 = torch.bfloat16


def layer_norm_fwd(x, residual, gamma, beta, sum_out, y, mean_rstd, rows, d, eps, y_bf16=None):
    _numel_ok(x, rows * d, "x"); _numel_ok(mean_rstd, rows * 2, "mean_rstd")
    res = None if residual is None else _chk(residual, "residual", F32)
    so = None if sum_out is None else _chk(sum_out, "sum_out", F32)
    if x.dtype == F32 and y_bf16 is None:
        _numel_ok(y, rows * d, "y")
        _call("pda_layer_norm_fwd", x, _chk(x, "x", F32), res, _chk(gamma, "gamma", F32), _chk(beta, "beta", F32), so,
              _chk(y, "y", F32), _chk(mean_rstd, "mean_rstd", F32), rows, d, float(eps))
        return 1
    yp = yb = None
    if y is not None:
        _numel_ok(y, rows * d, "y"); yp = _chk(y, "y", F32)
    if y_bf16 is not None:
        _numel_ok(y_bf16, rows * d, "y_bf16"); yb = _chk(y_bf16, "y_bf16", BF16)
    _call("pda_layer_norm_fwd_mixed", x, _chk(x, "x", x.dtype if x.dtype == BF16 else F32), int(x.dtype == BF16), res,
          _chk(gamma, "gamma", F32), _chk(beta, "beta", F32), so, yp, yb, _chk(mean_rstd, "mean_rstd", F32), rows, d, float(eps))
    return 1


def layer_norm_bwd(x, grad_y, gamma, mean_rstd, grad_x, grad_gamma, grad_beta, scratch, rows, d, grad_y2=None, grad_x_bf16=None):
    _numel_ok(x, rows * d, "x"); _numel_ok(grad_y, rows * d, "grad_y"); _numel_ok(grad_x, rows * d, "grad_x")
    g2 = None
    if grad_y2 is not None:
        _numel_ok(grad_y2, rows * d, "grad_y2")
        g2 = _chk(grad_y2, "grad_y2", BF16 if grad_y2.dtype == BF16 else F32)
    if grad_x_bf16 is not None or (grad_y2 is not None and grad_y2.dtype == BF16):
        gxb = None
        if grad_x_bf16 is not None:
            _numel_ok(grad_x_bf16, rows * d, "grad_x_bf16"); gxb = _chk(grad_x_bf16, "grad_x_bf16", BF16)
        _call("pda_layer_norm_bwd_mixed", x, _chk(x, "x", F32), _chk(grad_y, "grad_y", F32), g2,
              int(grad_y2 is not None and grad_y2.dtype == BF16), _chk(gamma, "gamma", F32), _chk(mean_rstd, "mean_rstd", F32),
              _chk(grad_x, "grad_x", F32), gxb, _chk(grad_gamma, "grad_gamma", F32), _chk(grad_beta, "grad_beta", F32),
              _chk(scratch, "scratch", torch.uint8), rows, d)
        return 1
    _call("pda_layer_norm_bwd", x, _chk(x, "x", F32), _chk(grad_y, "grad_y", F32), g2, _chk(gamma, "gamma", F32),
          _chk(mean_rstd, "mean_rstd", F32), _chk(grad_x, "grad_x", F32), _chk(grad_gamma, "grad_gamma", F32),
          _chk(grad_beta, "grad_beta", F32), _chk(scratch, "scratch", torch.uint8), rows, d)
    return 1


_WGRAD_SCRATCH_BYTES = {}


def _wgrad_scratch_bytes(tokens, in_features, out_features):
    key = (tokens, in_features, out_features)
    nbytes = _WGRAD_SCRATCH_BYTES.get(key)
    if nbytes is None:
        if len(_WGRAD_SCRATCH_BYTES) >= 4096:
            _WGRAD_SCRATCH_BYTES.clear()
        nbytes = _WGRAD_SCRATCH_BYTES[key] = int(_lib.load().pda_linear_wgrad_scratch_bytes(tokens, in_features, out_features))
    return nbytes


@functools.lru_cache(maxsize=None)
def _split_packed_bytes(n_out, k):
    return int(_lib.load().pda_linear_split_packed_bytes(n_out, k))


@functools.lru_cache(maxsize=None)
def _cols_packed_size(n_out, k):
    return int(_lib.load().pda_linear_cols_packed_size(n_out, k))


def linear_wgrad(x, grad_out, grad_weight, grad_bias, tokens, in_features, out_features):
    _numel_ok(x, tokens * in_features, "x"); _numel_ok(grad_out, tokens * out_features, "grad_out")
    _numel_ok(grad_weight, in_features * out_features, "grad_weight")
    nbytes = _wgrad_scratch_bytes(tokens, in_features, out_features)
    scratch = torch.empty((nbytes,), dtype=torch.uint8, device=x.device)
    gb = None if grad_bias is None else _chk(grad_bias, "grad_bias", F32)
    _call("pda_linear_wgrad", x, _chk(x, "x", F32), _chk(grad_out, "grad_out", F32), _chk(grad_weight, "grad_weight", F32),
          gb, _chk(scratch, "scratch", torch.uint8), tokens, in_features, out_features)
    return 1


def linear_wgrad_bn(x, grad_out, grad_weight, tokens, in_features, out_features, x_mean_invstd, x_gamma, x_beta):
    _numel_ok(x, tokens * in_features, "x"); _numel_ok(grad_out, tokens * out_features, "grad_out")
    _numel_ok(grad_weight, in_features * out_features, "grad_weight"); _numel_ok(x_mean_invstd, 2 * in_features, "x_mean_invstd")
    _numel_ok(x_gamma, in_features, "x_gamma"); _numel_ok(x_beta, in_features, "x_beta")
    nbytes = _wgrad_scratch_bytes(tokens, in_features, out_features)
    scratch = torch.empty((nbytes,), dtype=torch.uint8, device=x.device)
    _call("pda_linear_wgrad_bn", x, _chk(x, "x", F32), _chk(grad_out, "grad_out", F32), _chk(grad_weight, "grad_weight", F32), None,
          _chk(scratch, "scratch", torch.uint8), tokens, in_features, out_features, _chk(x_mean_invstd, "x_mean_invstd", F32),
          _chk(x_gamma, "x_gamma", F32), _chk(x_beta, "x_beta", F32))
    return 1


def gemm_split_bn_tiles(tokens):
    return (int(tokens) + 255) // 256


def gemm_split_bn(x, wf, y, tokens, k, n_out, in_bn=None, stats_mode=0, partial=None):
    _numel_ok(x, tokens * k, "x"); _numel_ok(y, tokens * n_out, "y")
    _numel_ok(wf, _split_packed_bytes(int(n_out), int(k)), "wf")
    ib = (None, None, None)
    if in_bn is not None:
        _numel_ok(in_bn[0], 2 * k, "in_mean_invstd"); _numel_ok(in_bn[1], k, "in_gamma"); _numel_ok(in_bn[2], k, "in_beta")
        ib = tuple(_chk(t, "in_bn", F32) for t in in_bn)
    if stats_mode:
        _numel_ok(partial, gemm_split_bn_tiles(tokens) * 2 * n_out, "partial")
    _call("pda_gemm_split_bn", x, _chk(x, "x", F32), _chk(wf, "wf", torch.uint8), _chk(y, "y", F32), tokens, k, n_out, ib[0], ib[1], ib[2],
          int(stats_mode), None if partial is None else _chk(partial, "partial", torch.float64))
    return 1


def gemm_split_maxpool(x, wf, bias, out, tokens, k, n_out, ns, relu=True):
    _numel_ok(x, tokens * k, "x"); _numel_ok(out, (tokens // ns) * n_out, "out")
    _numel_ok(wf, _split_packed_bytes(int(n_out), int(k)), "wf")
    if bias is not None:
        _numel_ok(bias, n_out, "bias")
    _call("pda_gemm_split_maxpool", x, _chk(x, "x", F32), _chk(wf, "wf", torch.uint8), None if bias is None else _chk(bias, "bias", F32),
          _chk(out, "out", F32), tokens, k, n_out, ns, 1 if relu else 0)
    return 1


def gemm_split_gather(point_rows, xyz, new_xyz, idx, w1, bias1, wf, bias2, y, b, n, m, ns, k, n_out, relu=True):
    t = b * m * ns
    _numel_ok(point_rows, b * n * k, "point_rows"); _numel_ok(xyz, b * n * 3, "xyz"); _numel_ok(new_xyz, b * m * 3, "new_xyz")
    _numel_ok(idx, t, "idx"); _numel_ok(y, t * n_out, "y"); _numel_ok(wf, _split_packed_bytes(int(n_out), int(k)), "wf")
    if w1.dim() != 2 or w1.shape[0] != k or w1.shape[1] < 3:
        raise RuntimeError("w1 must be (k, 3 + c)")
    _call("pda_gemm_split_gather", y, _chk(point_rows, "point_rows", F32), _chk(xyz, "xyz", F32), _chk(new_xyz, "new_xyz", F32),
          _chk(idx, "idx", I32), _chk(w1, "w1", F32), int(w1.shape[1]), None if bias1 is None else _chk(bias1, "bias1", F32),
          _chk(wf, "wf", torch.uint8), None if bias2 is None else _chk(bias2, "bias2", F32), _chk(y, "y", F32), b, n, m, ns, k, n_out,
          1 if relu else 0)
    return 1


def bn_stats_fwd(x, running_mean, running_var, mean_invstd, scratch, rows, c, eps, momentum):
    _numel_ok(x, rows * c, "x"); _numel_ok(mean_invstd, 2 * c, "mean_invstd")
    rm = None if running_mean is None else _chk(running_mean, "running_mean", F32)
    rv = None if running_var is None else _chk(running_var, "running_var", F32)
    _buffers_written(rm)
    _call("pda_bn_stats_fwd", x, _chk(x, "x", F32), rm, rv, _chk(mean_invstd, "mean_invstd", F32), _chk(scratch, "scratch", torch.uint8),
          rows, c, float(eps), float(momentum))
    return 1


def bn_finalize_fwd(partial, nblocks, c, count, eps, momentum, mean_invstd, running_mean, running_var):
    _numel_ok(partial, nblocks * 2 * c, "partial"); _numel_ok(mean_invstd, 2 * c, "mean_invstd")
    rm = None if running_mean is None else _chk(running_mean, "running_mean", F32)
    rv = None if running_var is None else _chk(running_var, "running_var", F32)
    _buffers_written(rm)
    _call("pda_bn_finalize_fwd", partial, _chk(partial, "partial", torch.float64), nblocks, c, count, float(eps), float(momentum),
          _chk(mean_invstd, "mean_invstd", F32), rm, rv)
    return 1


def bn_relu_max_pool_apply(x, gamma, beta, mean_invstd, out, arg, groups, ns, c):
    _numel_ok(x, groups * ns * c, "x"); _numel_ok(out, groups * c, "out"); _numel_ok(arg, groups * c, "arg"); _numel_ok(mean_invstd, 2 * c, "mean_invstd")
    _call("pda_bn_relu_max_pool_apply", x, _chk(x, "x", F32), _chk(gamma, "gamma", F32), _chk(beta, "beta", F32),
          _chk(mean_invstd, "mean_invstd", F32), _chk(out, "out", F32), _chk(arg, "arg", torch.uint8), groups, ns, c)
    return 1


def colsum_bf16(g, out, rows, cols):
    _numel_ok(g, rows * cols, "g"); _numel_ok(out, cols, "out")
    scratch = torch.empty((int(_lib.load().pda_colsum_scratch_bytes(cols)),), dtype=torch.uint8, device=g.device)
    _call("pda_colsum_bf16", g, _chk(g, "g", torch.bfloat16), _chk(out, "out", F32), _chk(scratch, "scratch", torch.uint8), rows, cols)
    return 1


@functools.lru_cache(maxsize=None)
def densitynet_sizes():
# ... 374 lines not shown
```

### pdanet_amd/pointnet2_utils.py

```python
from typing import List, Tuple

import os

import torch
import torch.nn as nn
from torch.autograd import Function

from . import _lib
from . import param_cache
from . import pointnet2_batch_cuda as pointnet2

_fwd = torch.amp.custom_fwd(device_type="cuda", cast_inputs=torch.float32)
_bwd = torch.amp.custom_bwd(device_type="cuda")


class FarthestPointSampling(Function):

    @staticmethod
    @_fwd
    def forward(ctx, xyz: torch.Tensor, npoint: int) -> torch.Tensor:
        assert xyz.is_contiguous()
        B, N, _ = xyz.size()
        output = torch.empty((B, npoint), dtype=torch.int32, device=xyz.device)
        temp = torch.full((B, N), 1e10, dtype=torch.float32, device=xyz.device)
        pointnet2.farthest_point_sampling_wrapper(B, N, npoint, xyz, temp, output)
        ctx.mark_non_differentiable(output)
        return output

    @staticmethod
    def backward(ctx, a=None):
        return None, None


farthest_point_sample = furthest_point_sample = FarthestPointSampling.apply


class FurthestPointSamplingWithDist(Function):

    @staticmethod
    @_fwd
    def forward(ctx, xyz: torch.Tensor, npoint: int) -> torch.Tensor:
        assert xyz.is_contiguous()
        B, N, _ = xyz.size()
        output = torch.empty((B, npoint), dtype=torch.int32, device=xyz.device)
        temp = torch.full((B, N), 1e10, dtype=torch.float32, device=xyz.device)
        pointnet2.furthest_point_sampling_with_dist_wrapper(B, N, npoint, xyz, temp, output)
        ctx.mark_non_differentiable(output)
        return output

    @staticmethod
    def backward(ctx, a=None):
        return None, None


furthest_point_sample_with_dist = FurthestPointSamplingWithDist.apply


class GatherOperation(Function):

    @staticmethod
    @_fwd
    def forward(ctx, features: torch.Tensor, idx: torch.Tensor) -> torch.Tensor:
        assert features.is_contiguous()
        assert idx.is_contiguous()
        B, npoint = idx.size()
        _, C, N = features.size()
        output = torch.empty((B, C, npoint), dtype=torch.float32, device=features.device)
        pointnet2.gather_points_wrapper(B, C, N, npoint, features, idx, output)
        ctx.for_backwards = (idx, C, N)
        return output

    @staticmethod
    @_bwd
    def backward(ctx, grad_out):
        idx, C, N = ctx.for_backwards
        B, npoint = idx.size()
        grad_features = torch.zeros((B, C, N), dtype=torch.float32, device=grad_out.device)
        grad_out_data = grad_out.detach().contiguous()
        pointnet2.gather_points_grad_wrapper(B, C, N, npoint, grad_out_data, idx, grad_features)
        return grad_features, None


gather_operation = GatherOperation.apply

# ... 323 lines not shown
        k = len(metas)
        xs, params = [x.contiguous() for x in flat[:k]], flat[k:]
        nparam, nscratch = pointnet2.densitynet_sizes()
        problems, saved, ys = [], [], []
        for i, (x, (eps, momentum, running, part)) in enumerate(zip(xs, metas)):
            packed = torch.cat([p.reshape(-1) for p in params[12 * i:12 * i + 12]])
            assert packed.numel() == nparam
            y = torch.empty_like(x)
            stats = torch.empty((46,), dtype=torch.float32, device=x.device)
            scratch = torch.empty((nscratch,), dtype=torch.uint8, device=x.device)
            prob = dict(x=x, params=packed, y=y, stats=stats, scratch=scratch, running=running, n=x.numel(), eps=eps, momentum=momentum)
            keep = [x, packed, stats]
            if part is not None:
                _, off, rowmap, roww, G, ns = part
                prob.update(rowmap=rowmap, roww=roww, off=off, groups=G, nsample=ns)
                keep += [off, rowmap, roww]
            problems.append(prob)
            saved.append((keep, None if part is None else (part[4], part[5]), eps))
            ys.append(y)
        pointnet2.densitynet_multi(problems)
        ctx.save_for_backward(*[t for keep, _, _ in saved for t in keep])
        ctx.layout = [(len(keep), uq, eps) for keep, uq, eps in saved]
        ctx.shapes = [p.shape for p in params]
        return tuple(ys)

    @staticmethod
    def backward(ctx, *grad_ys):
        nparam, nscratch = pointnet2.densitynet_sizes()
        tensors = list(ctx.saved_tensors)
        problems, grads = [], []
        for (cnt, uq, eps), gy in zip(ctx.layout, grad_ys):
            keep, tensors = tensors[:cnt], tensors[cnt:]
            x, packed, stats = keep[:3]
            g = torch.empty((nparam,), dtype=torch.float32, device=x.device)
            scratch = torch.empty((nscratch,), dtype=torch.uint8, device=x.device)
            gy = torch.zeros_like(x) if gy is None else gy.contiguous()
            prob = dict(x=x, grad_y=gy, params=packed, stats=stats, grad_params=g, scratch=scratch, n=x.numel(), eps=eps)
            if uq is not None:
                prob.update(off=keep[3], rowmap=keep[4], roww=keep[5], groups=uq[0], nsample=uq[1])
            problems.append(prob)
            grads.append(g)
        pointnet2.densitynet_multi(problems, backward=True)
        out = []
        for i, g in enumerate(grads):
            out += [t.view(s) for t, s in zip(torch.split(g, DensityNetFused.SPLITS), ctx.shapes[12 * i:12 * i + 12])]
        return (None,) + (None,) * len(grads) + tuple(out)


FUSED_DENSITYNET = True
DENSITYNET_MULTI = os.environ.get("PDA_DENSITYNET_MULTI", "1") != "0"
DENSITYNET_UNIQUE = os.environ.get("PDA_DENSITYNET_UNIQUE", "1") != "0"


def densitynet(dn, x, part=None):
    convs, bns = dn.mlp_convs, dn.mlp_bns
    running = None
    if all(b.track_running_stats for b in bns):
        running = [t for b in bns for t in (b.running_mean, b.running_var)]
        for b in bns:
            bump_bn_counter(b)
    params = []
    for c, b in zip(convs, bns):
        params += [c.weight, c.bias, b.weight, b.bias]
    return DensityNetFused.apply(x, bns[0].eps, bns[0].momentum, running, part if DENSITYNET_UNIQUE else None, *params)


def densitynet_multi(dns, xs, parts):
    if not DENSITYNET_MULTI or len(dns) == 1 or len(dns) > 4:
        return [densitynet(dn, x, part) for dn, x, part in zip(dns, xs, parts)]
    metas, params = [], []
    for dn, part in zip(dns, parts):
        convs, bns = dn.mlp_convs, dn.mlp_bns
        running = None
        if all(b.track_running_stats for b in bns):
            running = [t for b in bns for t in (b.running_mean, b.running_var)]
            for b in bns:
                bump_bn_counter(b)
        metas.append((bns[0].eps, bns[0].momentum, running, part if DENSITYNET_UNIQUE else None))
        for c, b in zip(convs, bns):
            params += [c.weight, c.bias, b.weight, b.bias]
    return list(DensityNetFusedMulti.apply(metas, *xs, *params))


class LinearLongTokens(Function):
    MIN_TOKENS = 4096
    SPLIT_MIN_TOKENS = 32768

    @staticmethod
    def supported(x, weight):
        return torch.is_grad_enabled() and not torch.is_autocast_enabled() and LinearLongTokens.kernel_wins(x, weight)

    @staticmethod
    def kernel_wins(x, weight):
        if not (x.is_cuda and x.dtype == torch.float32 and weight.dtype == torch.float32 and weight.dim() == 2):
            return False
        n_out, n_in = weight.shape
        tokens = x.numel() // max(1, x.shape[-1])
        if n_out % 4 or n_in % 4:
            return False
        if max(n_out, n_in) <= 64:
            return tokens >= 4096
        return min(n_out, n_in) >= 64 and tokens >= LinearLongTokens.MIN_TOKENS

    @staticmethod
    def forward(ctx, x, weight, bias):
        ctx.save_for_backward(x, weight)
        ctx.has_bias = bias is not None
        if x.numel() // x.shape[-1] < LinearLongTokens.SPLIT_MIN_TOKENS or min(weight.shape) < 128:
            return torch.nn.functional.linear(x, weight, bias)
        return _gemm_nt(x.reshape(-1, x.shape[-1]), weight, bias).view(*x.shape[:-1], weight.shape[0])

    @staticmethod
    def backward(ctx, grad_out):
        x, weight = ctx.saved_tensors
        grad_out = grad_out.contiguous()
        gx = gw = gb = None
        if ctx.needs_input_grad[0]:
            if grad_out.numel() // grad_out.shape[-1] < LinearLongTokens.SPLIT_MIN_TOKENS or min(weight.shape) < 128:
                gx = grad_out.matmul(weight)
            else:
                gx = _gemm_nn(grad_out.reshape(-1, grad_out.shape[-1]), weight).view(*grad_out.shape[:-1], weight.shape[1])
        if ctx.needs_input_grad[1] or (ctx.has_bias and ctx.needs_input_grad[2]):
            n_out, n_in = weight.shape
            xc = x.contiguous()
            tokens = xc.numel() // n_in
            gw = torch.empty_like(weight)
            gb = torch.empty((n_out,), dtype=torch.float32, device=x.device) if ctx.has_bias else None
            pointnet2.linear_wgrad(xc, grad_out, gw, gb, tokens, n_in, n_out)
        return gx, gw, gb


DENSE_BF16 = False
BF16_MIN_TOKENS = 32768
BF16_MIN_FEATURES = 128


def _dense_bf16(x, weight=None):
    if not (DENSE_BF16 and x.is_cuda and x.dtype in (torch.float32, torch.bfloat16) and not torch.is_autocast_enabled()):
        return False
    if x.numel() // max(1, x.shape[-1]) < BF16_MIN_TOKENS:
        return False
    return weight is None or min(weight.shape[0], weight.shape[1]) >= BF16_MIN_FEATURES


def _b16(t):
    return t if t.dtype == torch.bfloat16 else t.to(torch.bfloat16)


_B16_COPIES = param_cache.Store(under_capture=False)


def _b16p(p):
    if p.dtype == torch.bfloat16:
        return p

    def cast():
        return p.detach().to(torch.bfloat16)
    pb = _B16_COPIES.get(p, (p,), cast)
    return cast() if pb is None else pb


SPLIT_GEMM = os.environ.get("PDA_SPLIT_GEMM", "1") != "0"

SPLIT_GEMM_MIN_TOKENS = 4096


# ... 147 lines not shown
    S = 64
    while S > 16 and S * tiles > 768:
        S //= 2
    while S > 1 and (T % S or T // S < 512):
        S //= 2
    if S > 1:
        gw = torch.bmm(gb.view(S, T // S, n_out).transpose(1, 2), xb.view(S, T // S, n_in), out_dtype=torch.float32).sum(0)
    else:
        gw = torch.mm(gb.t(), xb, out_dtype=torch.float32)
    if not want_bias:
        return gw, None
    if n_out % 8 == 0 and n_out <= 2048 and gb.is_contiguous():
        gbias = torch.empty((n_out,), dtype=torch.float32, device=gb.device)
        pointnet2.colsum_bf16(gb, gbias, T, n_out)
        return gw, gbias
    return gw, gb.sum(0, dtype=torch.float32)


def _wgrad(x2d, g2d, weight, want_bias, bf16=False):
    if bf16:
        return _wgrad_bf16(_b16(x2d), _b16(g2d), want_bias)
    if LINEAR_WGRAD_KERNEL and LinearLongTokens.kernel_wins(x2d, weight):
        gw = torch.empty_like(weight)
        gb = torch.empty((weight.shape[0],), dtype=torch.float32, device=x2d.device) if want_bias else None
        pointnet2.linear_wgrad(x2d, g2d, gw, gb, x2d.shape[0], weight.shape[1], weight.shape[0])
        return gw, gb
    return g2d.t().mm(x2d), (g2d.sum(0) if want_bias else None)


class TransformerBlock(Function):

    @staticmethod
    def supported(x, heads):
        g, s_, d = x.shape
        return (LayerNormResidual.supported(x, d) and d % heads == 0 and s_ in GroupAttention.SUPPORTED_SEQ
                and d // heads in GroupAttention.SUPPORTED_HD and not torch.is_autocast_enabled())

    @staticmethod
    def forward(ctx, x, n1w, n1b, in_w, in_b, out_w, out_b, n2w, n2b, w1, b1, w2, b2, heads, eps1, eps2, pool):
        bf16 = _dense_bf16(x)
        x = x.contiguous()
        G, S, D = x.shape
        T, hd = G * S, D // heads
        dev = x.device
        f32 = dict(dtype=torch.float32, device=dev)
        src1, ssum, src2 = torch.empty_like(x), torch.empty_like(x), torch.empty_like(x)
        st1, st2 = torch.empty((T, 2), **f32), torch.empty((T, 2), **f32)
        lse = torch.empty((G, heads, S), **f32)
        if bf16:
            b16 = dict(dtype=torch.bfloat16, device=dev)
            src1_s, src2_s = torch.empty((T, D), **b16), torch.empty((T, D), **b16)
            pointnet2.layer_norm_fwd(x, None, n1w, n1b, None, src1, st1, T, D, eps1, y_bf16=src1_s)
            qkv = torch.addmm(_b16p(in_b), src1_s, _b16p(in_w).t())
            a_s = torch.empty((T, D), **b16)
            pointnet2.group_attention_fwd(qkv, a_s, lse, G, S, heads, hd)
            proj = torch.addmm(_b16p(out_b), a_s, _b16p(out_w).t())
            pointnet2.layer_norm_fwd(proj, src1, n2w, n2b, ssum, src2, st2, T, D, eps2, y_bf16=src2_s)
            del proj
            h = h_s = torch._addmm_activation(_b16p(b1), src2_s, _b16p(w1).t())
            ffn = torch.addmm(_b16p(b2), h, _b16p(w2).t()).view(G, S, D)
        else:
            pointnet2.layer_norm_fwd(x, None, n1w, n1b, None, src1, st1, T, D, eps1)
            qkv = _gemm_nt(src1.view(T, D), in_w, in_b).view(G, S, 3 * D)
            a = torch.empty((G, S, D), **f32)
            pointnet2.group_attention_fwd(qkv, a, lse, G, S, heads, hd)
            proj = _gemm_nt(a.view(T, D), out_w, out_b).view(G, S, D)
            pointnet2.layer_norm_fwd(proj, src1, n2w, n2b, ssum, src2, st2, T, D, eps2)
            del proj
            h = _gemm_nt(src2.view(T, D), w1, b1, relu=True).view(G, S, -1)
            ffn = _gemm_nt(h.view(T, -1), w2, b2).view(G, S, D)
            src1_s, a_s, src2_s, h_s = src1.view(T, D), a.view(T, D), src2.view(T, D), h.view(T, -1)
        if pool:
            y = torch.empty((G, D), **f32)
            arg = torch.empty((G, D), dtype=torch.uint8, device=dev)
            pointnet2.add_max_pool(src2, ffn, y, arg, G, S, D)
        else:
            y = src2 + ffn
            arg = torch.empty((0,), dtype=torch.uint8, device=dev)
        ctx.save_for_backward(x, st1, src1_s, qkv, lse, a_s, ssum, st2, src2_s, h, h_s, n1w, in_w, out_w, n2w, w1, w2, arg)
        ctx.heads, ctx.pool, ctx.bf16 = heads, pool, bf16
        return y

    @staticmethod
    def backward(ctx, dy):
        x, st1, src1_s, qkv, lse, a_s, ssum, st2, src2_s, h, h_s, n1w, in_w, out_w, n2w, w1, w2, arg = ctx.saved_tensors
        G, S, D = x.shape
        T, heads, bf16 = G * S, ctx.heads, ctx.bf16
        hd = D // heads
        dev = x.device
        f32 = dict(dtype=torch.float32, device=dev)
        b16 = dict(dtype=torch.bfloat16, device=dev)
        if ctx.pool:
            dy2 = torch.empty((T, D), **f32)
            dy_g = torch.empty((T, D), **b16) if bf16 else dy2
            pointnet2.max_pool_scatter(dy.contiguous(), arg, dy2, G, S, D, grad_x_bf16=dy_g if bf16 else None)
        else:
            dy2 = dy.contiguous().view(T, D)
            dy_g = _b16(dy2) if bf16 else dy2
        d_h = torch.mm(dy_g, _b16p(w2)) if bf16 else _gemm_nn(dy_g, w2)
        if bf16 and ctx.pool:
            gw2, gb2 = _wgrad(h_s, dy_g, w2, False, True)[0], dy.sum(0)
        else:
            gw2, gb2 = _wgrad(h_s, dy_g, w2, True, bf16)
        del dy_g
        d_h = torch.ops.aten.threshold_backward(d_h, h.view(T, -1), 0)
        gw1, gb1 = _wgrad(src2_s, d_h, w1, True, bf16)
        d_lin1 = torch.mm(d_h, _b16p(w1)) if bf16 else _gemm_nn(d_h, w1)
        del d_h
        d_s = torch.empty((T, D), **f32)
        ds_g = torch.empty((T, D), **b16) if bf16 else d_s
        gn2w, gn2b = torch.empty_like(n2w), torch.empty_like(n2w)
        scratch = torch.empty((pointnet2.layer_norm_scratch_bytes(D),), dtype=torch.uint8, device=dev)
        pointnet2.layer_norm_bwd(ssum, dy2, n2w, st2, d_s, gn2w, gn2b, scratch, T, D, grad_y2=d_lin1, grad_x_bf16=ds_g if bf16 else None)
        del d_lin1
        d_a = torch.mm(ds_g, _b16p(out_w)) if bf16 else _gemm_nn(d_s, out_w)
        gwo, gbo = _wgrad(a_s, ds_g, out_w, True, bf16)
        del ds_g
        dqkv = torch.empty_like(qkv)
        pointnet2.group_attention_bwd(qkv, d_a.view(G, S, D), lse, dqkv, G, S, heads, hd)
        del d_a
        dqkv2 = dqkv.view(T, 3 * D)
        gwi, gbi = _wgrad(src1_s, dqkv2, in_w, True, bf16)
        d_src1 = _mm_nn(dqkv2, in_w, True, acc=d_s) if bf16 else _gemm_nn(dqkv2, in_w, acc=d_s)
        del dqkv, dqkv2
        d_x = torch.empty_like(x)
        gn1w, gn1b = torch.empty_like(n1w), torch.empty_like(n1w)
        pointnet2.layer_norm_bwd(x, d_src1, n1w, st1, d_x, gn1w, gn1b, scratch, T, D)
        return d_x, gn1w, gn1b, gwi, gbi, gwo, gbo, gn2w, gn2b, gw1, gb1, gw2, gb2, None, None, None, None


def transformer_block(tr, x, pool=False):
    at = tr.self_attn
    return TransformerBlock.apply(x, tr.norm1.weight, tr.norm1.bias, at.in_proj_weight, at.in_proj_bias, at.out_proj.weight,
                                  at.out_proj.bias, tr.norm2.weight, tr.norm2.bias, tr.linear1.weight, tr.linear1.bias,
                                  tr.linear2.weight, tr.linear2.bias, at.num_heads, tr.norm1.eps, tr.norm2.eps, pool)


SA_MFMA_TRAIN = True
SA_MFMA_EVENTS = None


def _sa_timed(flops, fn, pipe="f32"):
    ev = SA_MFMA_EVENTS
    if ev is None or torch.cuda.is_current_stream_capturing():
        return fn()
    e0, e1 = torch.cuda.Event(enable_timing=True), torch.cuda.Event(enable_timing=True)
    e0.record()
    fn()
    e1.record()
    ev.append((e0, e1, flops, pipe))




def _lin_cols(x2, weight, y, T, k, n_out, transposed):
    if SPLIT_GEMM:
        wf = _split_planes(weight, transposed)
        if _rows_in_registers(T, k, n_out):
            _sa_timed(2.0 * T * k * n_out, lambda: pointnet2.linear_split(x2, wf, None, y, T, k, n_out), "bf16x6")
        else:
            _sa_timed(2.0 * T * k * n_out, lambda: pointnet2.gemm_split(x2, wf, None, y, T, k, n_out), "bf16x6")
    else:
        wf = pointnet2.linear_cols_pack(weight, n_out, k, transposed_source=transposed)
        _sa_timed(2.0 * T * k * n_out, lambda: pointnet2.linear_cols(x2, wf, y, T, k, n_out))


class LinearColsMFMA(Function):

    @staticmethod
    def supported(x, weight):
        n_out, k = weight.shape
        return (SA_MFMA_TRAIN and x.is_cuda and x.dtype == torch.float32 and weight.dtype == torch.float32 and k in (256, 512)
                and n_out % 128 == 0 and n_out <= 1024 and x.shape[-1] == k and not torch.is_autocast_enabled() and not DENSE_BF16)

    @staticmethod
    def forward(ctx, x, weight):
        n_out, k = weight.shape
        x2 = x.contiguous().view(-1, k)
        T = x2.shape[0]
        y = torch.empty((T, n_out), dtype=torch.float32, device=x.device)
        _lin_cols(x2, weight.contiguous(), y, T, k, n_out, False)
        ctx.save_for_backward(x2, weight)
        ctx.x_shape = x.shape
        return y.view(*x.shape[:-1], n_out)

    @staticmethod
    def backward(ctx, grad_out):
        x2, weight = ctx.saved_tensors
        n_out, k = weight.shape
        g2 = grad_out.contiguous().view(-1, n_out)
        T = g2.shape[0]
        gx = gw = None
        if ctx.needs_input_grad[0]:
            if n_out in (256, 512) and k % 128 == 0:
                gx = torch.empty((T, k), dtype=torch.float32, device=g2.device)
                _lin_cols(g2, weight.contiguous(), gx, T, n_out, k, True)
            else:
                gx = _gemm_nn(g2, weight)
            gx = gx.view(ctx.x_shape)
        if ctx.needs_input_grad[1]:
            gw = _wgrad(x2, g2, weight, False)[0]
        return gx, gw


class SaGatherLinear(Function):

    @staticmethod
    def supported(xyz, feats_pm, weight):
        return (SA_MFMA_TRAIN and xyz.is_cuda and feats_pm is not None and feats_pm.dtype == torch.float32 and feats_pm.shape[-1] == 256
                and weight.shape[1] == 259 and weight.shape[0] % 128 == 0 and weight.shape[0] <= 1024
# ... 195 lines not shown
def sa_small_chain_train(xyz, new_xyz, feats_pm, idx, mlp):
    layers = list(mlp)
    convs, bns = [layers[0], layers[3], layers[6]], [layers[1], layers[4], layers[7]]
    for bn in bns:
        bump_bn_counter(bn)
    return SaSmallChainTrain.apply(xyz, new_xyz, feats_pm, idx, convs[0].weight.flatten(1), convs[1].weight.flatten(1),
                                   convs[2].weight.flatten(1), bns[0].weight, bns[0].bias, bns[1].weight, bns[1].bias,
                                   bns[2].weight, bns[2].bias, bns)


SA_WIDE_CHAIN = os.environ.get("PDA_SA_WIDE_CHAIN", "1") != "0"
WIDE_CHAIN_DGRAD_FIRST = os.environ.get("PDA_WIDE_CHAIN_DGRAD_FIRST", "1") != "0"
SA_WIDE_FUSED_ENDS = os.environ.get("PDA_SA_WIDE_FUSED_ENDS", "1") != "0"
SA_WIDE_CHAIN_MIN_TOKENS = int(os.environ.get("PDA_SA_WIDE_CHAIN_MIN_TOKENS", "32768"))


class SaWideChainTrain(Function):

    @staticmethod
    def supported(xyz, new_xyz, feats_pm, idx, mlp):
        layers = list(mlp)
        if not (SA_WIDE_CHAIN and FUSED_WIDE_CHAIN_OK and len(layers) == 9 and feats_pm is not None and idx is not None):
            return False
        convs, bns = [layers[0], layers[3], layers[6]], [layers[1], layers[4], layers[7]]
        if not (all(isinstance(c, nn.Conv2d) and c.bias is None and c.weight.dtype == torch.float32 for c in convs)
                and all(isinstance(b, nn.BatchNorm2d) and b.affine and b.training and b.momentum is not None for b in bns)
                and all(isinstance(layers[k], nn.ReLU) for k in (2, 5, 8))):
            return False
        w1 = convs[0].weight.flatten(1)
        if not SaPointLinear.supported(xyz, feats_pm, w1):
            return False
        c1, c2, c3 = (c.weight.shape[0] for c in convs)
        T = idx.shape[0] * idx.shape[1] * idx.shape[2]
        if not (c1 % 256 == 0 and c2 % 256 == 0 and c3 % 256 == 0 and max(c1, c2, c3) <= 1024 and 1 <= idx.shape[2] <= 255
                and T >= SA_WIDE_CHAIN_MIN_TOKENS and not DENSE_BF16 and not torch.is_autocast_enabled()):
            return False
        lib = _lib.load()
        return int(lib.pda_linear_wgrad_form(T, c1, c2)) == 2 and int(lib.pda_linear_wgrad_form(T, c2, c3)) == 2

    @staticmethod
    def forward(ctx, xyz, new_xyz, feats_pm, idx, w1, w2, w3, g1, b1, g2, b2, g3, b3, bns):
        B, N, _ = xyz.shape
        M, ns = idx.shape[1], idx.shape[2]
        C, c1, c2, c3 = feats_pm.shape[-1], w1.shape[0], w2.shape[0], w3.shape[0]
        T = B * M * ns
        dev = xyz.device
        xyz, new_xyz, feats_pm, idx = xyz.contiguous(), new_xyz.contiguous(), feats_pm.contiguous(), idx.contiguous()
        gs = [t.detach().contiguous() for t in (g1, g2, g3)]
        bs = [t.detach().contiguous() for t in (b1, b2, b3)]
        stats = [(bn.running_mean, bn.running_var) if bn.track_running_stats else (None, None) for bn in bns]
        w1d = w1.detach().contiguous()
        rows = _gemm_nt(feats_pm.view(B * N, C), w1d[:, 3:].contiguous())
        z1 = torch.empty((T, c1), dtype=torch.float32, device=dev)
        mi1 = torch.empty((2 * c1,), dtype=torch.float32, device=dev)
        if SA_WIDE_FUSED_ENDS:
            nb1 = pointnet2.sa_point_gather_stats_blocks(T, c1)
            part1 = torch.empty((nb1 * 2 * c1,), dtype=torch.float64, device=dev)
            pointnet2.sa_point_gather_stats(rows, xyz, new_xyz, idx, w1d, z1, part1, B, N, M, ns, c1)
            pointnet2.bn_finalize_fwd(part1, nb1, c1, T, bns[0].eps, bns[0].momentum, mi1, stats[0][0], stats[0][1])
        else:
            pointnet2.sa_point_gather(rows, xyz, new_xyz, idx, w1d, z1, B, N, M, ns, c1)
            scratch = torch.empty((pointnet2.bn_relu_scratch_bytes(c1),), dtype=torch.uint8, device=dev)
            pointnet2.bn_stats_fwd(z1, stats[0][0], stats[0][1], mi1, scratch, T, c1, bns[0].eps, bns[0].momentum)
        tiles = pointnet2.gemm_split_bn_tiles(T)

        def layer(z_in, mi_in, k, w, n_out, bn, st, gi, bi):
            z = torch.empty((T, n_out), dtype=torch.float32, device=dev)
            part = torch.empty((tiles * 2 * n_out,), dtype=torch.float64, device=dev)
            wf = _split_planes(w)
            _sa_timed(2.0 * T * k * n_out, lambda: pointnet2.gemm_split_bn(z_in, wf, z, T, k, n_out, in_bn=(mi_in, gi, bi), stats_mode=1,
                                                                           partial=part), "bf16x6")
            mi = torch.empty((2 * n_out,), dtype=torch.float32, device=dev)
            pointnet2.bn_finalize_fwd(part, tiles, n_out, T, bn.eps, bn.momentum, mi, st[0], st[1])
            return z, mi
        z2, mi2 = layer(z1, mi1, c1, w2, c2, bns[1], stats[1], gs[0], bs[0])
        z3, mi3 = layer(z2, mi2, c2, w3, c3, bns[2], stats[2], gs[1], bs[1])
        out = torch.empty((B, M, c3), dtype=torch.float32, device=dev)
        arg = torch.empty((B, M, c3), dtype=torch.uint8, device=dev)
        pointnet2.bn_relu_max_pool_apply(z3, gs[2], bs[2], mi3, out, arg, B * M, ns, c3)
        ctx.save_for_backward(xyz, new_xyz, feats_pm, idx, w1, w2, w3, g1, b1, g2, b2, g3, b3, z1, z2, z3, mi1, mi2, mi3, arg)
        return out

    @staticmethod
    def backward(ctx, grad_out):
        xyz, new_xyz, feats_pm, idx, w1, w2, w3, g1, b1, g2, b2, g3, b3, z1, z2, z3, mi1, mi2, mi3, arg = ctx.saved_tensors
        B, M, ns = idx.shape
        N, C = xyz.shape[1], feats_pm.shape[-1]
        c1, c2, c3 = w1.shape[0], w2.shape[0], w3.shape[0]
        T = B * M * ns
        dev = xyz.device
        tiles = pointnet2.gemm_split_bn_tiles(T)
        with torch.no_grad():
            g1c, b1c, g2c, b2c, g3c, b3c = (t.contiguous() for t in (g1, b1, g2, b2, g3, b3))
            gz3 = torch.empty((T, c3), dtype=torch.float32, device=dev)
            dg3, db3 = torch.empty_like(g3c), torch.empty_like(b3c)
            scratch = torch.empty((pointnet2.bn_relu_scratch_bytes(c3),), dtype=torch.uint8, device=dev)
            pointnet2.bn_relu_max_pool_bwd(z3, grad_out.contiguous().float(), arg, g3c, b3c, mi3, gz3, dg3, db3, scratch, B * M, ns, c3)

            def layer(gz, w, z_in, mi_in, gi, bi, k_in, n_out, sums=None):
                dw = torch.empty((n_out, k_in), dtype=torch.float32, device=dev)
                ga = torch.empty((T, k_in), dtype=torch.float32, device=dev)
                if WIDE_CHAIN_DGRAD_FIRST:
                    _lin_cols(gz, w, ga, T, n_out, k_in, True)
                    pointnet2.linear_wgrad_bn(z_in, gz, dw, T, k_in, n_out, mi_in, gi, bi)
                else:
                    pointnet2.linear_wgrad_bn(z_in, gz, dw, T, k_in, n_out, mi_in, gi, bi)
                    _lin_cols(gz, w, ga, T, n_out, k_in, True)
                dg, db = torch.empty_like(gi), torch.empty_like(bi)
                scratch = torch.empty((pointnet2.bn_relu_scratch_bytes(k_in),), dtype=torch.uint8, device=dev)
                if sums is not None:
                    pointnet2.bn_relu_bwd_reduce(z_in, ga, gi, bi, mi_in, dg, db, sums, scratch, T, k_in)
                else:
                    pointnet2.bn_relu_bwd(z_in, ga, gi, bi, mi_in, ga, dg, db, scratch, T, k_in)
                return dw, ga, dg, db
            dw3, gz2, dg2, db2 = layer(gz3, w3, z2, mi2, g2c, b2c, c2, c3)
            del gz3
            sums1 = torch.empty((2 * c1,), dtype=torch.float32, device=dev) if SA_WIDE_FUSED_ENDS else None
            dw2, gz1, dg1, db1 = layer(gz2, w2, z1, mi1, g1c, b1c, c1, c2, sums1)
            del gz2
            w1c = w1.contiguous()
            dw1 = torch.empty_like(w1c)
            g_new = torch.empty_like(new_xyz) if ctx.needs_input_grad[1] else None
            if SA_WIDE_FUSED_ENDS:
                g_pts = torch.empty((B, N, c1), dtype=torch.float32, device=dev)
                pointnet2.sa_point_grad_bn(gz1, z1, mi1, g1c, b1c, sums1, xyz, new_xyz, idx, w1c, dw1, g_new, g_pts, B, N, M, ns, c1)
            else:
                pointnet2.sa_xyz_grad(gz1, xyz, new_xyz, idx, w1c, dw1, g_new, B, N, M, ns, c1)
                g_pts = torch.zeros((B, N, c1), dtype=torch.float32, device=dev)
                pointnet2.group_rows_grad(B, N, c1, M * ns, gz1, idx, g_pts)
            g_pts = g_pts.view(B * N, c1)
            dw1[:, 3:] = _wgrad(feats_pm.view(B * N, C), g_pts, torch.empty((c1, C), dtype=torch.float32, device=dev), False)[0]
            g_feats = _gemm_nn(g_pts, w1c[:, 3:].contiguous()).view(B, N, C) if ctx.needs_input_grad[2] else None
        return None, g_new, g_feats, None, dw1, dw2, dw3, dg1, db1, dg2, db2, dg3, db3, None


def sa_wide_chain_train(xyz, new_xyz, feats_pm, idx, mlp):
    layers = list(mlp)
    convs, bns = [layers[0], layers[3], layers[6]], [layers[1], layers[4], layers[7]]
    for bn in bns:
        bump_bn_counter(bn)
    return SaWideChainTrain.apply(xyz, new_xyz, feats_pm, idx, convs[0].weight.flatten(1), convs[1].weight.flatten(1),
                                  convs[2].weight.flatten(1), bns[0].weight, bns[0].bias, bns[1].weight, bns[1].bias,
                                  bns[2].weight, bns[2].bias, bns)


RAGGED_TOKENS = True
RAGGED_MAX_FRACTION = 0.85


class RaggedPlan:
    __slots__ = ("cnt", "off", "rowmap", "roww", "tokens", "groups", "nsample")

    def __init__(self, cnt, off, rowmap, roww, tokens, groups, nsample):
        self.cnt, self.off, self.rowmap, self.roww = cnt, off, rowmap, roww
        self.tokens, self.groups, self.nsample = tokens, groups, nsample

    @property
    def fraction(self):
        return self.tokens / float(self.groups * self.nsample)


def ragged_plan_parts(idxs):
    parts = []
    for idx in idxs:
        G, ns = idx.shape[0] * idx.shape[1], idx.shape[2]
        cnt = torch.empty((G,), dtype=torch.int32, device=idx.device)
        off = torch.empty((G + 1,), dtype=torch.int32, device=idx.device)
        rowmap = torch.empty((G * ns,), dtype=torch.int32, device=idx.device)
        roww = torch.empty((G * ns,), dtype=torch.float32, device=idx.device)
        pointnet2.ragged_plan(idx, cnt, off, rowmap, G, ns, roww)
        parts.append((cnt, off, rowmap, roww, G, ns))
    return parts, torch.stack([p[1][-1] for p in parts])


def ragged_plans_from(parts, totals):
    return [RaggedPlan(c, o, r[:u], w[:u], int(u), G, ns) for (c, o, r, w, G, ns), u in zip(parts, totals)]


def ragged_plans(idxs):
    parts, totals = ragged_plan_parts(idxs)
    return ragged_plans_from(parts, totals.tolist())


ASSEMBLE_BWD_TOKEN_PARALLEL = os.environ.get("PDA_ASSEMBLE_BWD_TOKEN_PARALLEL", "1") != "0"


class AssembleTokensRagged(Function):

    @staticmethod
    def forward(ctx, rppe, dscale, feats_pm, idx, glob, plan):
        B, M, ns = idx.shape
        C, N = feats_pm.shape[-1], feats_pm.shape[1]
        compact = rppe.dim() == 2
        rppe, dscale, feats_pm, glob = rppe.contiguous(), dscale.contiguous(), feats_pm.contiguous(), glob.contiguous()
        out = torch.empty((plan.tokens, 4 * C), dtype=torch.float32, device=rppe.device)
        pointnet2.assemble_tokens_ragged(rppe, dscale, feats_pm, idx, glob, plan.rowmap, plan.off, out, plan.tokens, B, N, M, ns, C,
                                         rppe_compact=compact)
        ctx.save_for_backward(dscale, feats_pm, idx, plan.cnt, plan.off, plan.rowmap)
        ctx.dims = (B, N, M, ns, C, plan.tokens, compact)
        return out

    @staticmethod
    def backward(ctx, grad_out):
        dscale, feats_pm, idx, cnt, off, rowmap = ctx.saved_tensors
        B, N, M, ns, C, U, compact = ctx.dims
        dev = grad_out.device
        g_rppe = torch.empty((U, C) if compact else (B, M, ns, C), dtype=torch.float32, device=dev)
        g_ds = torch.empty_like(dscale)
        g_feats = torch.zeros((B, N, C), dtype=torch.float32, device=dev)
        g_glob = torch.empty((B, M, C), dtype=torch.float32, device=dev)
        pointnet2.assemble_tokens_ragged_grad(grad_out.contiguous(), dscale, feats_pm, idx, cnt, off, g_rppe, g_ds, g_feats, g_glob,
                                              U, B, N, M, ns, C, rppe_compact=compact,
                                              rowmap=rowmap if ASSEMBLE_BWD_TOKEN_PARALLEL else None)
        return g_rppe, g_ds, g_feats, None, g_glob, None
# ... 21 lines not shown
        x, weight, bias, stats, roww = ctx.saved_tensors
        rows, c = x.shape
        gx = torch.empty_like(x)
        gw, gb = torch.empty_like(weight), torch.empty_like(bias)
        scratch = torch.empty((pointnet2.bn_relu_scratch_bytes(c),), dtype=torch.uint8, device=x.device)
        pointnet2.bn_relu_bwd_weighted(x, grad_y.contiguous(), weight, bias, stats, gx, gw, gb, scratch, rows, c, roww, ctx.count)
        return gx, gw, gb, None, None, None, None, None, None


def position_mlp_ragged_supported(layers, rppe):
    layers = list(layers)
    ok = (RAGGED_POSITION_MLP and rppe.is_cuda and rppe.dtype == torch.float32 and len(layers) == 6 and torch.is_grad_enabled()
          and not DENSE_BF16 and not torch.is_autocast_enabled())
    if not ok:
        return False
    for conv, bn in ((layers[0], layers[1]), (layers[3], layers[4])):
        c = conv.weight.shape[0]
        if (conv.bias is not None or not bn.training or not bn.affine or bn.momentum is None or c < 4 or c > 1024
                or (c & (c - 1)) != 0):
            return False
    return True


def position_mlp_ragged(layers, rppe, plan):
    layers = list(layers)
    x = rppe.reshape(-1, rppe.shape[-1]).index_select(0, plan.rowmap)
    count = plan.groups * plan.nsample
    for conv, bn in ((layers[0], layers[1]), (layers[3], layers[4])):
        x = linear(x, conv.weight.flatten(1), None)
        rm, rv = (bn.running_mean, bn.running_var) if bn.track_running_stats else (None, None)
        bump_bn_counter(bn)
        x = BatchNormReLUWeighted.apply(x, bn.weight, bn.bias, rm, rv, bn.eps, bn.momentum, plan.roww, count)
    return x


def _wgrad_ragged(x2d, g2d, weight, want_bias):
    n_out, n_in = weight.shape
    tokens = x2d.shape[0]
    if (LINEAR_WGRAD_KERNEL and tokens >= 4096 and (min(n_out, n_in) >= 64 or max(n_out, n_in) <= 64) and n_out % 4 == 0
            and n_in % 4 == 0 and x2d.dtype == torch.float32 and g2d.dtype == torch.float32):
        gw = torch.empty_like(weight)
        gb = torch.empty((n_out,), dtype=torch.float32, device=x2d.device) if want_bias else None
        pointnet2.linear_wgrad(x2d.contiguous(), g2d.contiguous(), gw, gb, tokens, n_in, n_out)
        return gw, gb
    return g2d.t().mm(x2d), (g2d.sum(0) if want_bias else None)


class RaggedTransformerBlock(Function):

    @staticmethod
    def supported(d, heads, nsample, x):
        return (RAGGED_TOKENS and x.is_cuda and x.dtype == torch.float32 and d in (256, 512, 1024) and d % heads == 0
                and nsample in GroupAttention.SUPPORTED_SEQ and d // heads in GroupAttention.SUPPORTED_HD
                and not torch.is_autocast_enabled() and not DENSE_BF16)

    @staticmethod
    def forward(ctx, x, plan, n1w, n1b, in_w, in_b, out_w, out_b, n2w, n2b, w1, b1, w2, b2, heads, eps1, eps2):
        x = x.contiguous()
        U, D = x.shape
        G, S, hd = plan.groups, plan.nsample, D // heads
        dev = x.device
        f32 = dict(dtype=torch.float32, device=dev)
        src1, ssum, src2 = torch.empty_like(x), torch.empty_like(x), torch.empty_like(x)
        st1, st2 = torch.empty((U, 2), **f32), torch.empty((U, 2), **f32)
        lse = torch.empty((G, heads, S), **f32)
        pointnet2.layer_norm_fwd(x, None, n1w, n1b, None, src1, st1, U, D, eps1)
        qkv = _gemm_nt(src1, in_w, in_b)
        a = torch.empty((U, D), **f32)
        pointnet2.group_attention_ragged_fwd(qkv, plan.cnt, plan.off, a, lse, U, G, S, heads, hd)
        proj = _gemm_nt(a, out_w, out_b)
        pointnet2.layer_norm_fwd(proj, src1, n2w, n2b, ssum, src2, st2, U, D, eps2)
        del proj
        h = _gemm_nt(src2, w1, b1, relu=True)
        ffn = _gemm_nt(h, w2, b2)
        y = torch.empty((G, D), **f32)
        arg = torch.empty((G, D), dtype=torch.uint8, device=dev)
        pointnet2.add_max_pool_ragged(src2, ffn, plan.cnt, plan.off, y, arg, U, G, D)
        ctx.save_for_backward(x, st1, src1, qkv, lse, a, ssum, st2, src2, h, n1w, in_w, out_w, n2w, w1, w2, arg,
                              plan.cnt, plan.off, plan.rowmap)
        ctx.heads, ctx.dims = heads, (G, S)
        return y

    @staticmethod
    def backward(ctx, dy):
        x, st1, src1, qkv, lse, a, ssum, st2, src2, h, n1w, in_w, out_w, n2w, w1, w2, arg, cnt, off, rowmap = ctx.saved_tensors
        U, D = x.shape
        G, S = ctx.dims
        heads = ctx.heads
        hd = D // heads
        dev = x.device
        f32 = dict(dtype=torch.float32, device=dev)
        dy2 = torch.empty((U, D), **f32)
        pointnet2.max_pool_scatter_ragged(dy.contiguous(), arg, rowmap, off, dy2, U, G, S, D)
        d_h = _gemm_nn(dy2, w2)
        gw2, gb2 = _wgrad_ragged(h, dy2, w2, True)
        d_h = torch.ops.aten.threshold_backward(d_h, h, 0)
        gw1, gb1 = _wgrad_ragged(src2, d_h, w1, True)
        d_lin1 = _gemm_nn(d_h, w1)
        del d_h
        d_s = torch.empty((U, D), **f32)
        gn2w, gn2b = torch.empty_like(n2w), torch.empty_like(n2w)
        scratch = torch.empty((pointnet2.layer_norm_scratch_bytes(D),), dtype=torch.uint8, device=dev)
        pointnet2.layer_norm_bwd(ssum, dy2, n2w, st2, d_s, gn2w, gn2b, scratch, U, D, grad_y2=d_lin1)
        del d_lin1
        d_a = _gemm_nn(d_s, out_w)
        gwo, gbo = _wgrad_ragged(a, d_s, out_w, True)
        dqkv = torch.empty_like(qkv)
        pointnet2.group_attention_ragged_bwd(qkv, d_a, lse, cnt, off, dqkv, U, G, S, heads, hd)
        del d_a
        gwi, gbi = _wgrad_ragged(src1, dqkv, in_w, True)
        d_src1 = _gemm_nn(dqkv, in_w, acc=d_s)
        del dqkv
        d_x = torch.empty_like(x)
        gn1w, gn1b = torch.empty_like(n1w), torch.empty_like(n1w)
        pointnet2.layer_norm_bwd(x, d_src1, n1w, st1, d_x, gn1w, gn1b, scratch, U, D)
        return d_x, None, gn1w, gn1b, gwi, gbi, gwo, gbo, gn2w, gn2b, gw1, gb1, gw2, gb2, None, None, None


def ragged_transformer_block(tr, x, plan):
    at = tr.self_attn
    return RaggedTransformerBlock.apply(x, plan, tr.norm1.weight, tr.norm1.bias, at.in_proj_weight, at.in_proj_bias,
                                        at.out_proj.weight, at.out_proj.bias, tr.norm2.weight, tr.norm2.bias,
                                        tr.linear1.weight, tr.linear1.bias, tr.linear2.weight, tr.linear2.bias,
                                        at.num_heads, tr.norm1.eps, tr.norm2.eps)


class LayerNormResidual(Function):

    @staticmethod
    def supported(x, d):
        return x.is_cuda and x.dtype == torch.float32 and x.shape[-1] == d and d in (256, 512, 1024) and x.numel() > 0

    @staticmethod
    def forward(ctx, x, residual, weight, bias, eps):
        x = x.contiguous()
        d = x.shape[-1]
        rows = x.numel() // d
        y = torch.empty_like(x)
        stats = torch.empty((rows, 2), dtype=torch.float32, device=x.device)
        if residual is not None:
            s = torch.empty_like(x)
            pointnet2.layer_norm_fwd(x, residual.contiguous(), weight, bias, s, y, stats, rows, d, eps)
        else:
            s = x
            pointnet2.layer_norm_fwd(x, None, weight, bias, None, y, stats, rows, d, eps)
        ctx.save_for_backward(s, weight, stats)
        ctx.has_residual = residual is not None
        return y

    @staticmethod
    def backward(ctx, grad_y):
        s, weight, stats = ctx.saved_tensors
        d = s.shape[-1]
        rows = s.numel() // d
        gx = torch.empty_like(s)
        gw, gb = torch.empty_like(weight), torch.empty_like(weight)
        scratch = torch.empty((pointnet2.layer_norm_scratch_bytes(d),), dtype=torch.uint8, device=s.device)
        pointnet2.layer_norm_bwd(s, grad_y.contiguous(), weight, stats, gx, gw, gb, scratch, rows, d)
        return gx, (gx if ctx.has_residual else None), gw, gb, None


def layer_norm(x, ln, residual=None):
    return LayerNormResidual.apply(x, residual, ln.weight, ln.bias, ln.eps)


class BallQuery(Function):

    @staticmethod
    @_fwd
    def forward(ctx, radius: float, nsample: int, xyz: torch.Tensor, new_xyz: torch.Tensor) -> torch.Tensor:
        assert new_xyz.is_contiguous()
        assert xyz.is_contiguous()
        B, N, _ = xyz.size()
        npoint = new_xyz.size(1)
        idx = torch.zeros((B, npoint, nsample), dtype=torch.int32, device=xyz.device)
        pointnet2.ball_query_wrapper(B, N, npoint, radius, nsample, new_xyz, xyz, idx)
        ctx.mark_non_differentiable(idx)
        return idx

    @staticmethod
    def backward(ctx, a=None):
        return None, None, None, None


ball_query = BallQuery.apply


class BallQueryDilated(Function):

    @staticmethod
    @_fwd
    def forward(ctx, max_radius: float, min_radius: float, nsample: int, xyz: torch.Tensor,
                new_xyz: torch.Tensor) -> torch.Tensor:
        assert new_xyz.is_contiguous()
        assert xyz.is_contiguous()
        B, N, _ = xyz.size()
        npoint = new_xyz.size(1)
        idx = torch.zeros((B, npoint, nsample), dtype=torch.int32, device=xyz.device)
# ... 157 lines not shown
```

Measured before the change: 123.4 scenes/s.

## Batch parameter-gradient reductions per backward into one grouped reduce launch

Inside the transformer-block and SA-module backward passes, weight-gradient and layer-norm gamma/beta gradient kernels now write only their per-slice partials. A single grouped kernel then reduces all of them, replacing many small finalize/reduce launches with one. It also adds a float4-vectorised wgrad reduce path, enabled by default through an env flag, and lets dw1 be written straight into a strided column block. In exchange, scratch buffers must stay alive until the group closes, which raises memory use, and the thread-local grouping adds host-side bookkeeping.

Result: faster. 127.2 scenes/s (median of 6 runs) (+3.1%).

```diff
diff --git a/include/pda_train.h b/include/pda_train.h
--- a/include/pda_train.h
+++ b/include/pda_train.h
@@ -63,6 +63,24 @@
 int pda_linear_wgrad_bn(const float *x, const float *grad_out, float *grad_weight, float *grad_bias, void *scratch,
                         int64_t tokens, int in_features, int out_features, const float *x_mean_invstd,
                         const float *x_gamma, const float *x_beta, pda_stream_t stream);
+
+typedef struct pda_param_grad_entry {
+    int32_t kind, count;
+    const float *part, *part_bias;
+    float *dst, *dst_bias;
+    int64_t nm;
+    int32_t n, cols;
+    int64_t ld;
+} pda_param_grad_entry_t;
+int pda_linear_wgrad_partials(const float *x, const float *grad_out, void *scratch, int want_bias, int64_t tokens,
+                              int in_features, int out_features, int *slices, pda_stream_t stream);
+int pda_linear_wgrad_bn_partials(const float *x, const float *grad_out, void *scratch, int64_t tokens, int in_features,
+                                 int out_features, const float *x_mean_invstd, const float *x_gamma,
+                                 const float *x_beta, int *slices, pda_stream_t stream);
+int pda_layer_norm_bwd_partials(const float *x, const float *grad_y, const void *grad_y2, int grad_y2_is_bf16,
+                                const float *gamma, const float *mean_rstd, float *grad_x, uint16_t *grad_x_bf16,
+                                void *scratch, int64_t rows, int d, int *nblocks, pda_stream_t stream);
+int pda_param_grad_reduce_grouped(const pda_param_grad_entry_t *entries, int n, pda_stream_t stream);
 
 int64_t pda_gemm_split_bn_tiles(int64_t tokens);
 int pda_gemm_split_bn(const float *x, const void *wf, float *y, int64_t tokens, int k, int n_out,
diff --git a/pdanet_amd/_lib.py b/pdanet_amd/_lib.py
--- a/pdanet_amd/_lib.py
+++ b/pdanet_amd/_lib.py
@@ -28,6 +28,12 @@
                                                "dt_name", "dt_start", "dt_count", "ov_start", "frame_mode")] + \
                [("n_gt_total", ctypes.c_int64), ("det_cap", ctypes.c_int64), ("ov_cap", ctypes.c_int64),
                 ("n_frames", ctypes.c_int), ("max_gt", ctypes.c_int), ("max_det", ctypes.c_int)]
+
+
+class ParamGradEntry(ctypes.Structure):
+    _fields_ = [("kind", ctypes.c_int32), ("count", ctypes.c_int32), ("part", ctypes.c_void_p), ("part_bias", ctypes.c_void_p),
+                ("dst", ctypes.c_void_p), ("dst_bias", ctypes.c_void_p), ("nm", ctypes.c_int64), ("n", ctypes.c_int32),
+                ("cols", ctypes.c_int32), ("ld", ctypes.c_int64)]
 
 
 PARAM_EPOCH = [0]
@@ -93,6 +99,10 @@
     "pda_linear_wgrad_form": [ctypes.c_int64, _i, _i],
     "pda_linear_wgrad": [_vp, _vp, _vp, _vp, _vp, ctypes.c_int64, _i, _i, _vp],
     "pda_linear_wgrad_bn": [_vp, _vp, _vp, _vp, _vp, ctypes.c_int64, _i, _i, _vp, _vp, _vp, _vp],
+    "pda_linear_wgrad_partials": [_vp, _vp, _vp, _i, ctypes.c_int64, _i, _i, ctypes.POINTER(_i), _vp],
+    "pda_linear_wgrad_bn_partials": [_vp, _vp, _vp, ctypes.c_int64, _i, _i, _vp, _vp, _vp, ctypes.POINTER(_i), _vp],
+    "pda_layer_norm_bwd_partials": [_vp, _vp, _vp, _i, _vp, _vp, _vp, _vp, _vp, ctypes.c_int64, _i, ctypes.POINTER(_i), _vp],
+    "pda_param_grad_reduce_grouped": [ctypes.POINTER(ParamGradEntry), _i, _vp],
     "pda_gemm_split_bn_tiles": [ctypes.c_int64],
     "pda_gemm_split_bn": [_vp, _vp, _vp, ctypes.c_int64, _i, _i, _vp, _vp, _vp, _i, _vp, _vp],
     "pda_gemm_split_maxpool": [_vp, _vp, _vp, _vp, ctypes.c_int64, _i, _i, _i, _i, _vp],
diff --git a/pdanet_amd/csrc/layer_norm.hip b/pdanet_amd/csrc/layer_norm.hip
--- a/pdanet_amd/csrc/layer_norm.hip
+++ b/pdanet_amd/csrc/layer_norm.hip
@@ -1,4 +1,5 @@
 #include "pda_common.h"
+#include "param_grad_reduce.h"
 
 namespace pda {
 
@@ -119,30 +120,7 @@
 __global__ __launch_bounds__(1024) void layer_norm_finalize_kernel(const float* __restrict__ partial, int nblocks, int d,
                                                                    float* __restrict__ dgamma, float* __restrict__ dbeta) {
     __shared__ float red[2][16][64];
-    const int cl = threadIdx.x & 63, part = threadIdx.x >> 6;
-    const int c = blockIdx.x * 64 + cl;
-    float a = 0.f, b = 0.f;
-    if (c < d) {
-        float va[8], vb[8];
-        for (int k0 = part; k0 < nblocks; k0 += 16 * 8) {
-#pragma unroll
-            for (int u = 0; u < 8; ++u) {
-                const int k = k0 + 16 * u;
-                va[u] = k < nblocks ? partial[((size_t)k * 2 + 0) * d + c] : 0.f;
-                vb[u] = k < nblocks ? partial[((size_t)k * 2 + 1) * d + c] : 0.f;
-            }
-#pragma unroll
-            for (int u = 0; u < 8; ++u) { a += va[u]; b += vb[u]; }
-        }
-    }
-    red[0][part][cl] = a; red[1][part][cl] = b;
-    __syncthreads();
-    if (part != 0 || c >= d) return;
-    float s1 = 0.f, s2 = 0.f;
-#pragma unroll
-    for (int p = 0; p < 16; ++p) { s1 += red[0][p][cl]; s2 += red[1][p][cl]; }
-    dbeta[c] = s1;
-    dgamma[c] = s2;
+    layer_norm_finalize_block(partial, nblocks, d, dgamma, dbeta, (int)blockIdx.x, red);
 }
 
 static int ln_grid(int64_t rows) {
@@ -179,10 +157,10 @@
 template <typename T2>
 static int launch_layer_norm_bwd(const float* x, const float* grad_y, const T2* grad_y2, const float* gamma, const float* mean_rstd,
                                  float* grad_x, bf16_t* grad_x_b, float* grad_gamma, float* grad_beta, void* scratch, int64_t rows, int d,
-                                 hipStream_t st, const char* what) {
+                                 hipStream_t st, const char* what, int* nblocks_out = nullptr) {
     PDA_REQUIRE(rows >= 1, "%s: rows = %lld", what, (long long)rows);
     PDA_REQUIRE(d == 256 || d == 512 || d == 1024, "%s: D = %d (256, 512 or 1024)", what, d);
-    PDA_REQUIRE(x && grad_y && gamma && mean_rstd && grad_x && grad_gamma && grad_beta && scratch, "%s: null pointer", what);
+    PDA_REQUIRE(x && grad_y && gamma && mean_rstd && grad_x && ((grad_gamma && grad_beta) || nblocks_out) && scratch, "%s: null pointer", what);
     PDA_REQUIRE((((uintptr_t)x | (uintptr_t)grad_y | (uintptr_t)grad_x | (uintptr_t)gamma) & 15) == 0 &&
                     ((uintptr_t)grad_y2 & (4 * sizeof(T2) - 1)) == 0 && ((uintptr_t)grad_x_b & 7) == 0,
                 "%s: pointers must be 16-byte aligned (8 for bf16 tensors)", what);
@@ -194,7 +172,8 @@
     else hipLaunchKernelGGL((layer_norm_bwd_kernel<V, false, T2>), grid, block, 0, st, x, grad_y, grad_y2, gamma, mean_rstd, grad_x, grad_x_b, partial, rows)
     if (d == 256) { PDA_LN_BWD(1); } else if (d == 512) { PDA_LN_BWD(2); } else { PDA_LN_BWD(4); }
 #undef PDA_LN_BWD
-    hipLaunchKernelGGL(layer_norm_finalize_kernel, dim3(divup(d, 64)), dim3(1024), 0, st, partial, nblocks, d, grad_gamma, grad_beta);
+    if (nblocks_out) *nblocks_out = nblocks;
+    else hipLaunchKernelGGL(layer_norm_finalize_kernel, dim3(divup(d, 64)), dim3(1024), 0, st, partial, nblocks, d, grad_gamma, grad_beta);
     return check_launch(what);
 }
 
@@ -232,6 +211,19 @@
                                                        grad_gamma, grad_beta, scratch, rows, d, (hipStream_t)stream, "pda_layer_norm_bwd_mixed");
     return pda::launch_layer_norm_bwd<float>(x, grad_y, (const float*)grad_y2, gamma, mean_rstd, grad_x, grad_x_bf16, grad_gamma, grad_beta,
                                              scratch, rows, d, (hipStream_t)stream, "pda_layer_norm_bwd_mixed");
+}
+
+PDA_API int pda_layer_norm_bwd_partials(const float* x, const float* grad_y, const void* grad_y2, int grad_y2_is_bf16, const float* gamma,
+                                        const float* mean_rstd, float* grad_x, uint16_t* grad_x_bf16, void* scratch, int64_t rows, int d,
+                                        int* nblocks, pda_stream_t stream) {
+    PDA_REQUIRE(rows >= 1 && (d == 256 || d == 512 || d == 1024), "pda_layer_norm_bwd_partials: bad size: rows=%lld D=%d (256, 512 or 1024)",
+                (long long)rows, d);
+    PDA_REQUIRE(nblocks, "pda_layer_norm_bwd_partials: null pointer");
+    if (grad_y2_is_bf16)
+        return pda::launch_layer_norm_bwd<pda::bf16_t>(x, grad_y, (const pda::bf16_t*)grad_y2, gamma, mean_rstd, grad_x, grad_x_bf16, nullptr,
+                                                       nullptr, scratch, rows, d, (hipStream_t)stream, "pda_layer_norm_bwd_partials", nblocks);
+    return pda::launch_layer_norm_bwd<float>(x, grad_y, (const float*)grad_y2, gamma, mean_rstd, grad_x, grad_x_bf16, nullptr, nullptr, scratch,
+                                             rows, d, (hipStream_t)stream, "pda_layer_norm_bwd_partials", nblocks);
 }
 
 namespace pda {
diff --git a/pdanet_amd/csrc/param_grad_reduce.h b/pdanet_amd/csrc/param_grad_reduce.h
--- /dev/null
+++ b/pdanet_amd/csrc/param_grad_reduce.h
@@ -0,0 +1,117 @@
+#pragma once
+#include "pda_common.h"
+
+namespace pda {
+
+__device__ __forceinline__ float sum_slices(const float* __restrict__ part, int S, int64_t stride, int64_t e, bool live, int slice,
+                                            float (*red)[64], int el) {
+    float a = 0.f;
+    if (live) {
+        float v[8];
+        for (int s0 = slice; s0 < S; s0 += 16 * 8) {
+#pragma unroll
+            for (int u = 0; u < 8; ++u) {
+                const int sidx = s0 + 16 * u;
+                v[u] = sidx < S ? part[(size_t)sidx * stride + e] : 0.f;
+            }
+#pragma unroll
+            for (int u = 0; u < 8; ++u) a += v[u];
+        }
+    }
+    red[slice][el] = a;
+    __syncthreads();
+    float r = 0.f;
+    if (slice == 0)
+#pragma unroll
+        for (int p = 0; p < 16; ++p) r += red[p][el];
+    __syncthreads();
+    return r;
+}
+
+__device__ __forceinline__ void wgrad_reduce_block(const float* __restrict__ part_w, const float* __restrict__ part_b,
+                                                   float* __restrict__ dw, float* __restrict__ db, int S, int64_t nm, int N,
+                                                   int cols, int64_t ld, int blk, float (*red)[64]) {
+    const int el = threadIdx.x & 63, slice = threadIdx.x >> 6;
+    const int64_t e = (int64_t)blk * 64 + el;
+    const float w = sum_slices(part_w, S, nm, e, e < nm, slice, red, el);
+    if (slice == 0 && e < nm) dw[ld == cols ? e : (e / cols) * ld + e % cols] = w;
+    if (db && (int64_t)blk * 64 < N) {
+        const float bsum = sum_slices(part_b, S, N, e, e < N, slice, red, el);
+        if (slice == 0 && e < N) db[e] = bsum;
+    }
+}
+
+__device__ __forceinline__ float sum_slices4(const float* __restrict__ part, int S, int64_t stride, int64_t e4, bool live, int slice,
+                                             float (*red)[256], int q) {
+    float4 a = make_float4(0.f, 0.f, 0.f, 0.f);
+    if (live) {
+        float4 v[8];
+        for (int s0 = slice; s0 < S; s0 += 16 * 8) {
+#pragma unroll
+            for (int u = 0; u < 8; ++u) {
+                const int sidx = s0 + 16 * u;
+                v[u] = sidx < S ? *reinterpret_cast<const float4*>(part + (size_t)sidx * stride + e4) : make_float4(0.f, 0.f, 0.f, 0.f);
+            }
+#pragma unroll
+            for (int u = 0; u < 8; ++u) { a.x += v[u].x; a.y += v[u].y; a.z += v[u].z; a.w += v[u].w; }
+        }
+    }
+    *reinterpret_cast<float4*>(&red[slice][4 * q]) = a;
+    __syncthreads();
+    float r = 0.f;
+    if (threadIdx.x < 256)
+#pragma unroll
+        for (int p = 0; p < 16; ++p) r += red[p][threadIdx.x];
+    __syncthreads();
+    return r;
+}
+
+__host__ __device__ __forceinline__ bool wgrad_reduce_vec_ok(const float* part_w, const float* part_b, int64_t nm, int N) {
+    return (nm & 3) == 0 && (N & 3) == 0 && (((uintptr_t)part_w | (uintptr_t)part_b) & 15) == 0;
+}
+
+__device__ __forceinline__ void wgrad_reduce_block4(const float* __restrict__ part_w, const float* __restrict__ part_b,
+                                                    float* __restrict__ dw, float* __restrict__ db, int S, int64_t nm, int N,
+                                                    int cols, int64_t ld, int blk, float (*red)[256]) {
+    const int q = threadIdx.x & 63, slice = threadIdx.x >> 6;
+    const int64_t e4 = (int64_t)blk * 256 + 4 * q, e = (int64_t)blk * 256 + threadIdx.x;
+    const float w = sum_slices4(part_w, S, nm, e4, e4 < nm, slice, red, q);
+    if (threadIdx.x < 256 && e < nm) dw[ld == cols ? e : (e / cols) * ld + e % cols] = w;
+    if (db && (int64_t)blk * 256 < N) {
+        const float bsum = sum_slices4(part_b, S, N, e4, e4 < N, slice, red, q);
+        if (threadIdx.x < 256 && e < N) db[e] = bsum;
+    }
+}
+
+__device__ __forceinline__ void layer_norm_finalize_block(const float* __restrict__ partial, int nblocks, int d,
+                                                          float* __restrict__ dgamma, float* __restrict__ dbeta, int blk,
+                                                          float (*red)[16][64]) {
+    const int cl = threadIdx.x & 63, part = threadIdx.x >> 6;
+    const int c = blk * 64 + cl;
+    float a = 0.f, b = 0.f;
+    if (c < d) {
+        float va[8], vb[8];
+        for (int k0 = part; k0 < nblocks; k0 += 16 * 8) {
+#pragma unroll
+            for (int u = 0; u < 8; ++u) {
+                const int k = k0 + 16 * u;
+                va[u] = k < nblocks ? partial[((size_t)k * 2 + 0) * d + c] : 0.f;
+                vb[u] = k < nblocks ? partial[((size_t)k * 2 + 1) * d + c] : 0.f;
+            }
+#pragma unroll
+            for (int u = 0; u < 8; ++u) { a += va[u]; b += vb[u]; }
+        }
+    }
+    red[0][part][cl] = a; red[1][part][cl] = b;
+    __syncthreads();
+    if (part != 0 || c >= d) return;
+    float s1 = 0.f, s2 = 0.f;
+#pragma unroll
+    for (int p = 0; p < 16; ++p) { s1 += red[0][p][cl]; s2 += red[1][p][cl]; }
+    dbeta[c] = s1;
+    dgamma[c] = s2;
+}
+
+constexpr int PARAM_GRAD_WEIGHT = 0, PARAM_GRAD_LAYER_NORM = 1;
+
+}
diff --git a/pdanet_amd/csrc/wgrad.hip b/pdanet_amd/csrc/wgrad.hip
--- a/pdanet_amd/csrc/wgrad.hip
+++ b/pdanet_amd/csrc/wgrad.hip
@@ -1,5 +1,6 @@
 #include "pda_common.h"
 #include "split_bf16.h"
+#include "param_grad_reduce.h"
 
 #include <stdlib.h>
 
@@ -332,42 +333,17 @@
     }
 }
 
-__device__ __forceinline__ float sum_slices(const float* __restrict__ part, int S, int64_t stride, int64_t e, bool live, int slice,
-                                            float (*red)[64], int el) {
-    float a = 0.f;
-    if (live) {
-        float v[8];
-        for (int s0 = slice; s0 < S; s0 += 16 * 8) {
-#pragma unroll
-            for (int u = 0; u < 8; ++u) {
-                const int sidx = s0 + 16 * u;
-                v[u] = sidx < S ? part[(size_t)sidx * stride + e] : 0.f;
-            }
-#pragma unroll
-            for (int u = 0; u < 8; ++u) a += v[u];
-        }
-    }
-    red[slice][el] = a;
-    __syncthreads();
-    float r = 0.f;
-    if (slice == 0)
-#pragma unroll
-        for (int p = 0; p < 16; ++p) r += red[p][el];
-    __syncthreads();
-    return r;
-}
-
+template <bool VEC>
 __global__ __launch_bounds__(1024) void wgrad_reduce_kernel(const float* __restrict__ part_w, const float* __restrict__ part_b,
                                                             float* __restrict__ dw, float* __restrict__ db, int S, int64_t nm, int N) {
-    __shared__ float red[16][64];
-    const int el = threadIdx.x & 63, slice = threadIdx.x >> 6;
-    const int64_t e = (int64_t)blockIdx.x * 64 + el;
-    const float w = sum_slices(part_w, S, nm, e, e < nm, slice, red, el);
-    if (slice == 0 && e < nm) dw[e] = w;
-    if (db && (int64_t)blockIdx.x * 64 < N) {
-        const float bsum = sum_slices(part_b, S, N, e, e < N, slice, red, el);
-        if (slice == 0 && e < N) db[e] = bsum;
-    }
+    __shared__ __attribute__((aligned(16))) float red[VEC ? 16 * 256 : 16 * 64];
+    if constexpr (VEC) wgrad_reduce_block4(part_w, part_b, dw, db, S, nm, N, 1, 1, (int)blockIdx.x, reinterpret_cast<float (*)[256]>(red));
+    else wgrad_reduce_block(part_w, part_b, dw, db, S, nm, N, 1, 1, (int)blockIdx.x, reinterpret_cast<float (*)[64]>(red));
+}
+
+static bool wgrad_reduce_vec(const float* part_w, const float* part_b, int64_t nm, int N) {
+    static const bool on = [] { const char* e = getenv("PDA_WGRAD_REDUCE_VEC"); return !e || atoi(e) != 0; }();
+    return on && wgrad_reduce_vec_ok(part_w, part_b, nm, N);
 }
 
 constexpr int WS_UNROLL = 8;
@@ -503,12 +479,38 @@
 
 namespace pda {
 static int linear_wgrad(const float* x, const float* grad_out, float* grad_weight, float* grad_bias, void* scratch, int64_t tokens,
-                        int in_features, int out_features, pda_stream_t stream, const float* x_mi, const float* x_g, const float* x_b);
+                        int in_features, int out_features, pda_stream_t stream, const float* x_mi, const float* x_g, const float* x_b,
+                        int* slices = nullptr, bool want_bias = false);
 }
 
 PDA_API int pda_linear_wgrad(const float* x, const float* grad_out, float* grad_weight, float* grad_bias, void* scratch,
                              int64_t tokens, int in_features, int out_features, pda_stream_t stream) {
     return pda::linear_wgrad(x, grad_out, grad_weight, grad_bias, scratch, tokens, in_features, out_features, stream, nullptr, nullptr, nullptr);
+}
+
+PDA_API int pda_linear_wgrad_partials(const float* x, const float* grad_out, void* scratch, int want_bias, int64_t tokens,
+                                      int in_features, int out_features, int* slices, pda_stream_t stream) {
+    PDA_REQUIRE(tokens >= 1 && in_features >= 4 && out_features >= 4 && (in_features & 3) == 0 && (out_features & 3) == 0,
+                "pda_linear_wgrad_partials: bad size: tokens=%lld in=%d out=%d (features must be multiples of 4)", (long long)tokens,
+                in_features, out_features);
+    PDA_REQUIRE(slices, "pda_linear_wgrad_partials: null pointer");
+    return pda::linear_wgrad(x, grad_out, nullptr, nullptr, scratch, tokens, in_features, out_features, stream, nullptr, nullptr, nullptr,
+                             slices, want_bias != 0);
+}
+
+PDA_API int pda_linear_wgrad_bn_partials(const float* x, const float* grad_out, void* scratch, int64_t tokens, int in_features,
+                                         int out_features, const float* x_mean_invstd, const float* x_gamma, const float* x_beta,
+                                         int* slices, pda_stream_t stream) {
+    PDA_REQUIRE(tokens >= 1 && in_features >= 4 && out_features >= 4 && (in_features & 3) == 0 && (out_features & 3) == 0,
+                "pda_linear_wgrad_bn_partials: bad size: tokens=%lld in=%d out=%d (features must be multiples of 4)", (long long)tokens,
+                in_features, out_features);
+    if (pda_linear_wgrad_form(tokens, in_features, out_features) != 2) {
+        pda::set_error("pda_linear_wgrad_bn_partials: tokens=%lld in=%d out=%d does not run on the split form", (long long)tokens, in_features, out_features);
+        return PDA_ERR_UNSUPPORTED;
+    }
+    PDA_REQUIRE(x_mean_invstd && x_gamma && x_beta && slices, "pda_linear_wgrad_bn_partials: null pointer");
+    return pda::linear_wgrad(x, grad_out, nullptr, nullptr, scratch, tokens, in_features, out_features, stream, x_mean_invstd, x_gamma, x_beta,
+                             slices, false);
 }
 
 PDA_API int pda_linear_wgrad_bn(const float* x, const float* grad_out, float* grad_weight, float* grad_bias, void* scratch,
@@ -523,19 +525,32 @@
 }
 
 int pda::linear_wgrad(const float* x, const float* grad_out, float* grad_weight, float* grad_bias, void* scratch, int64_t tokens,
-                             int in_features, int out_features, pda_stream_t stream, const float* x_mi, const float* x_g, const float* x_b) {
+                             int in_features, int out_features, pda_stream_t stream, const float* x_mi, const float* x_g, const float* x_b,
+                             int* slices, bool want_bias) {
     const int M = in_features, N = out_features;
     PDA_REQUIRE(tokens >= 1 && M >= 4 && N >= 4 && (M & 3) == 0 && (N & 3) == 0,
                 "pda_linear_wgrad: tokens=%lld in=%d out=%d (features must be multiples of 4)", (long long)tokens, M, N);
-    PDA_REQUIRE(x && grad_out && grad_weight && scratch, "pda_linear_wgrad: null pointer");
+    PDA_REQUIRE(x && grad_out && (grad_weight || slices) && scratch, "pda_linear_wgrad: null pointer");
     PDA_REQUIRE((((uintptr_t)x | (uintptr_t)grad_out) & 15) == 0, "pda_linear_wgrad: x / grad_out must be 16-byte aligned");
+    const bool bias = slices ? want_bias : grad_bias != nullptr;
     int tm, tn, S;
     int64_t KS;
     hipStream_t st = (hipStream_t)stream;
+    const int64_t nm = (int64_t)N * M;
+    auto finish = [&](const float* part_w, const float* part_b) {
+        if (slices) *slices = S;
+        else if (pda::wgrad_reduce_vec(part_w, part_b, nm, N))
+            hipLaunchKernelGGL(pda::wgrad_reduce_kernel<true>, dim3((unsigned)pda::divup64(nm, 256)), dim3(1024), 0, st, part_w, part_b,
+                               grad_weight, grad_bias, S, nm, N);
+        else
+            hipLaunchKernelGGL(pda::wgrad_reduce_kernel<false>, dim3((unsigned)pda::divup64(nm, 64)), dim3(1024), 0, st, part_w, part_b,
+                               grad_weight, grad_bias, S, nm, N);
+        return pda::check_launch("pda_linear_wgrad");
+    };
     if (pda::wgrad_is_skinny(M, N)) {
         pda::wgrad_skinny_plan(tokens, S, KS);
         float* pw = (float*)scratch;
-        float* pb = grad_bias ? pw + (size_t)S * N * M : (float*)nullptr;
+        float* pb = bias ? pw + (size_t)S * N * M : (float*)nullptr;
         const int nt = N > 32 ? 2 : 1, mt = M > 32 ? 2 : 1;
 #define PDA_WS_CASE(A, B) hipLaunchKernelGGL((pda::wgrad_skinny_kernel<A, B>), dim3(S), dim3(256), 0, st, x, grad_out, pw, pb, tokens, M, N, KS)
         if (nt == 1 && mt == 1) PDA_WS_CASE(1, 1);
@@ -543,10 +558,7 @@
         else if (mt == 1) PDA_WS_CASE(2, 1);
         else PDA_WS_CASE(2, 2);
 #undef PDA_WS_CASE
-        const int64_t nm = (int64_t)N * M;
-        hipLaunchKernelGGL(pda::wgrad_reduce_kernel, dim3((unsigned)pda::divup64(nm, 64)), dim3(1024), 0, st, pw, pb, grad_weight,
-                           grad_bias, S, nm, N);
-        return pda::check_launch("pda_linear_wgrad");
+        return finish(pw, pb);
     }
     if (pda::wgrad_use_split(tokens, M, N)) {
         pda::wgrad_split_plan(tokens, M, N, tm, tn, S, KS);
@@ -560,25 +572,95 @@
         PDA_REQUIRE(ok, "pda_linear_wgrad: %d bytes of dynamic LDS refused", 2 * pda::WSP_TILE_U4 * 16);
         if (x_mi)
             hipLaunchKernelGGL(pda::wgrad_split_kernel<true>, dim3(pda::divup(nblocks, 8) * 8), dim3(512), 2 * pda::WSP_TILE_U4 * 16, st,
-                               x, grad_out, part_w, grad_bias ? part_b : (float*)nullptr, tokens, M, N, tm, tn, S, KS, nblocks, x_mi, x_g, x_b);
+                               x, grad_out, part_w, bias ? part_b : (float*)nullptr, tokens, M, N, tm, tn, S, KS, nblocks, x_mi, x_g, x_b);
         else
             hipLaunchKernelGGL(pda::wgrad_split_kernel<false>, dim3(pda::divup(nblocks, 8) * 8), dim3(512), 2 * pda::WSP_TILE_U4 * 16, st,
-                               x, grad_out, part_w, grad_bias ? part_b : (float*)nullptr, tokens, M, N, tm, tn, S, KS, nblocks, x_mi, x_g, x_b);
-        const int64_t nm = (int64_t)N * M;
-        hipLaunchKernelGGL(pda::wgrad_reduce_kernel, dim3((unsigned)pda::divup64(nm, 64)), dim3(1024), 0, st, part_w, part_b,
-                           grad_weight, grad_bias, S, nm, N);
-        return pda::check_launch("pda_linear_wgrad");
+                               x, grad_out, part_w, bias ? part_b : (float*)nullptr, tokens, M, N, tm, tn, S, KS, nblocks, x_mi, x_g, x_b);
+        return finish(part_w, part_b);
     }
     pda::wgrad_plan(tokens, M, N, tm, tn, S, KS);
     const int nblocks = S * tm * tn;
     float* part_w = (float*)scratch;
     float* part_b = part_w + (size_t)S * N * M;
     hipLaunchKernelGGL(pda::wgrad_kernel, dim3(pda::divup(nblocks, 8) * 8), dim3(256), 0, st, x, grad_out, part_w,
-                       grad_bias ? part_b : (float*)nullptr, tokens, M, N, tm, tn, S, KS, nblocks);
-    const int64_t nm = (int64_t)N * M;
-    hipLaunchKernelGGL(pda::wgrad_reduce_kernel, dim3((unsigned)pda::divup64(nm, 64)), dim3(1024), 0, st, part_w, part_b, grad_weight,
-                       grad_bias, S, nm, N);
-    return pda::check_launch("pda_linear_wgrad");
+                       bias ? part_b : (float*)nullptr, tokens, M, N, tm, tn, S, KS, nblocks);
+    return finish(part_w, part_b);
+}
+
+namespace pda {
+
+constexpr int PG_MAX_ENTRIES = 48;
+
+struct ParamGradArgs {
+    pda_param_grad_entry_t e[PG_MAX_ENTRIES];
+    int first[PG_MAX_ENTRIES + 1];
+    int n;
+    int vec;
+};
+
+static int param_grad_blocks(const pda_param_grad_entry_t& en, bool vec) {
+    if (en.kind != PARAM_GRAD_WEIGHT) return divup(en.n, 64);
+    return (int)divup64(en.nm, vec && wgrad_reduce_vec_ok(en.part, en.part_bias, en.nm, en.n) ? 256 : 64);
+}
+
+__global__ __launch_bounds__(1024) void param_grad_reduce_grouped_kernel(const ParamGradArgs a) {
+    __shared__ __attribute__((aligned(16))) float red[16 * 256];
+    const int b = (int)blockIdx.x;
+    int lo = 0, hi = a.n;
+    while (hi - lo > 1) {
+        const int mid = (lo + hi) >> 1;
+        if (a.first[mid] <= b) lo = mid; else hi = mid;
+    }
+    const pda_param_grad_entry_t& en = a.e[lo];
+    const int blk = b - a.first[lo];
+    if (en.kind != PARAM_GRAD_WEIGHT)
+        layer_norm_finalize_block(en.part, en.count, en.n, en.dst, en.dst_bias, blk, reinterpret_cast<float (*)[16][64]>(red));
+    else if (a.vec && wgrad_reduce_vec_ok(en.part, en.part_bias, en.nm, en.n))
+        wgrad_reduce_block4(en.part, en.part_bias, en.dst, en.dst_bias, en.count, en.nm, en.n, en.cols, en.ld, blk,
+                            reinterpret_cast<float (*)[256]>(red));
+    else
+        wgrad_reduce_block(en.part, en.part_bias, en.dst, en.dst_bias, en.count, en.nm, en.n, en.cols, en.ld, blk,
+                           reinterpret_cast<float (*)[64]>(red));
+}
+
+}
+
+PDA_API int pda_param_grad_reduce_grouped(const pda_param_grad_entry_t* entries, int n, pda_stream_t stream) {
+    PDA_REQUIRE(n >= 1, "pda_param_grad_reduce_grouped: bad size: n=%d", n);
+    PDA_REQUIRE(entries, "pda_param_grad_reduce_grouped: null pointer");
+    for (int i = 0; i < n; ++i) {
+        const pda_param_grad_entry_t& en = entries[i];
+        PDA_REQUIRE(en.kind == pda::PARAM_GRAD_WEIGHT || en.kind == pda::PARAM_GRAD_LAYER_NORM,
+                    "pda_param_grad_reduce_grouped: bad size: entry %d: kind=%d", i, en.kind);
+        PDA_REQUIRE(en.count >= 1 && en.n >= 1, "pda_param_grad_reduce_grouped: bad size: entry %d: count=%d n=%d", i, en.count, en.n);
+        if (en.kind == pda::PARAM_GRAD_WEIGHT)
+            PDA_REQUIRE(en.cols >= 1 && en.nm >= en.n && en.nm == (int64_t)en.n * en.cols && en.nm <= ((int64_t)1 << 30) && en.ld >= en.cols,
+                        "pda_param_grad_reduce_grouped: bad size: entry %d: nm=%lld n=%d cols=%d ld=%lld", i, (long long)en.nm, en.n, en.cols,
+                        (long long)en.ld);
+        else
+            PDA_REQUIRE(en.n <= 4096, "pda_param_grad_reduce_grouped: bad size: entry %d: d=%d", i, en.n);
+        PDA_REQUIRE(en.part && en.dst && (en.kind == pda::PARAM_GRAD_WEIGHT ? (en.dst_bias == nullptr || en.part_bias != nullptr) : en.dst_bias != nullptr),
+                    "pda_param_grad_reduce_grouped: entry %d: null pointer", i);
+    }
+    hipStream_t st = (hipStream_t)stream;
+    for (int i0 = 0; i0 < n; i0 += pda::PG_MAX_ENTRIES) {
+        pda::ParamGradArgs a;
+        a.n = n - i0 < pda::PG_MAX_ENTRIES ? n - i0 : pda::PG_MAX_ENTRIES;
+        a.vec = pda::wgrad_reduce_vec(nullptr, nullptr, 0, 0) ? 1 : 0;
+        int blocks = 0;
+        for (int i = 0; i < pda::PG_MAX_ENTRIES; ++i) {
+            a.first[i] = blocks;
+            if (i < a.n) {
+                a.e[i] = entries[i0 + i];
+                blocks += pda::param_grad_blocks(a.e[i], a.vec != 0);
+            } else {
+                a.e[i] = pda_param_grad_entry_t{};
+            }
+        }
+        a.first[pda::PG_MAX_ENTRIES] = blocks;
+        hipLaunchKernelGGL(pda::param_grad_reduce_grouped_kernel, dim3((unsigned)blocks), dim3(1024), 0, st, a);
+    }
+    return pda::check_launch("pda_param_grad_reduce_grouped");
 }
 
 namespace pda {
diff --git a/pdanet_amd/pointnet2_batch_cuda.py b/pdanet_amd/pointnet2_batch_cuda.py
--- a/pdanet_amd/pointnet2_batch_cuda.py
+++ b/pdanet_amd/pointnet2_batch_cuda.py
@@ -1,6 +1,8 @@
 import ctypes
 
 import functools
+import os
+import threading
 
 import torch
 
@@ -350,12 +352,92 @@
     return 1
 
 
+WGRAD_GROUPED = os.environ.get("PDA_WGRAD_GROUPED", "1") != "0"
+_TLS = threading.local()
+GROUP_STATS = {"grouped_calls": 0, "entries": 0, "partial_bytes": 0}
+
+
+class param_grad_group:
+    def __init__(self):
+        self.entries, self.keep = [], []
+
+    def __enter__(self):
+        if WGRAD_GROUPED and _open_group() is None:
+            _TLS.group = self
+        return self
+
+    def __exit__(self, exc_type, exc, tb):
+        if _open_group() is self:
+            _TLS.group = None
+            if exc_type is None:
+                self.flush()
+            self.entries, self.keep = [], []
+        return False
+
+    def add(self, entry, *tensors):
+        self.entries.append(entry)
+        self.keep.extend(tensors)
+
+    def flush(self):
+        if not self.entries:
+            return
+        arr = (_lib.ParamGradEntry * len(self.entries))(*self.entries)
+        _call("pda_param_grad_reduce_grouped", self.keep[0], arr, len(self.entries))
+        GROUP_STATS["grouped_calls"] += 1
+        GROUP_STATS["entries"] += len(self.entries)
+        GROUP_STATS["partial_bytes"] += sum(4 * e.count * (e.nm + e.n if e.part_bias else e.nm) if e.kind == 0 else 8 * e.count * e.n
+                                            for e in self.entries)
+        self.entries, self.keep = [], []
+
+
+def _open_group():
+    return getattr(_TLS, "group", None)
+
+
+def param_grad_group_open():
+    return _open_group() is not None
+
+
+def _grad_dst(t, name, rows, cols):
+    if not (isinstance(t, torch.Tensor) and t.is_cuda and t.dtype == F32):
+        raise RuntimeError("%s must be a float32 CUDA(HIP) tensor" % name)
+    if t.is_contiguous():
+        _numel_ok(t, rows * cols, name)
+        return t.data_ptr(), cols
+    if t.dim() != 2 or t.shape[0] != rows or t.shape[1] != cols or t.stride(1) != 1 or t.stride(0) < cols:
+        raise RuntimeError("%s must be contiguous or a (%d, %d) column block of a row-major matrix" % (name, rows, cols))
+    return t.data_ptr(), t.stride(0)
+
+
+def _wgrad_entry(scratch, slices, grad_weight, grad_bias, in_features, out_features):
+    nm = in_features * out_features
+    dst, ld = _grad_dst(grad_weight, "grad_weight", out_features, in_features)
+    part = scratch.data_ptr()
+    gb = None if grad_bias is None else _chk(grad_bias, "grad_bias", F32)
+    return _lib.ParamGradEntry(0, slices, part, part + 4 * slices * nm if gb is not None else None, dst, gb, nm, out_features,
+                               in_features, ld)
+
+
 def layer_norm_bwd(x, grad_y, gamma, mean_rstd, grad_x, grad_gamma, grad_beta, scratch, rows, d, grad_y2=None, grad_x_bf16=None):
     _numel_ok(x, rows * d, "x"); _numel_ok(grad_y, rows * d, "grad_y"); _numel_ok(grad_x, rows * d, "grad_x")
     g2 = None
     if grad_y2 is not None:
         _numel_ok(grad_y2, rows * d, "grad_y2")
         g2 = _chk(grad_y2, "grad_y2", BF16 if grad_y2.dtype == BF16 else F32)
+    group = _open_group()
+    if group is not None:
+        gxb = None
+        if grad_x_bf16 is not None:
+            _numel_ok(grad_x_bf16, rows * d, "grad_x_bf16"); gxb = _chk(grad_x_bf16, "grad_x_bf16", BF16)
+        _numel_ok(scratch, layer_norm_scratch_bytes(d), "scratch")
+        nblocks = ctypes.c_int(0)
+        _call("pda_layer_norm_bwd_partials", x, _chk(x, "x", F32), _chk(grad_y, "grad_y", F32), g2,
+              int(grad_y2 is not None and grad_y2.dtype == BF16), _chk(gamma, "gamma", F32), _chk(mean_rstd, "mean_rstd", F32),
+              _chk(grad_x, "grad_x", F32), gxb, _chk(scratch, "scratch", torch.uint8), rows, d, ctypes.byref(nblocks))
+        _numel_ok(grad_gamma, d, "grad_gamma"); _numel_ok(grad_beta, d, "grad_beta")
+        group.add(_lib.ParamGradEntry(1, nblocks.value, scratch.data_ptr(), None, _chk(grad_gamma, "grad_gamma", F32),
+                                       _chk(grad_beta, "grad_beta", F32), 0, d, 0, 0), scratch, grad_gamma, grad_beta)
+        return 1
     if grad_x_bf16 is not None or (grad_y2 is not None and grad_y2.dtype == BF16):
         gxb = None
         if grad_x_bf16 is not None:
@@ -396,9 +478,18 @@
 
 def linear_wgrad(x, grad_out, grad_weight, grad_bias, tokens, in_features, out_features):
     _numel_ok(x, tokens * in_features, "x"); _numel_ok(grad_out, tokens * out_features, "grad_out")
-    _numel_ok(grad_weight, in_features * out_features, "grad_weight")
     nbytes = _wgrad_scratch_bytes(tokens, in_features, out_features)
     scratch = torch.empty((nbytes,), dtype=torch.uint8, device=x.device)
+    group = _open_group()
+    if group is not None:
+        if grad_bias is not None:
+            _numel_ok(grad_bias, out_features, "grad_bias")
+        slices = ctypes.c_int(0)
+        _call("pda_linear_wgrad_partials", x, _chk(x, "x", F32), _chk(grad_out, "grad_out", F32), scratch.data_ptr(),
+              int(grad_bias is not None), tokens, in_features, out_features, ctypes.byref(slices))
+        group.add(_wgrad_entry(scratch, slices.value, grad_weight, grad_bias, in_features, out_features), scratch, grad_weight, grad_bias)
+        return 1
+    _numel_ok(grad_weight, in_features * out_features, "grad_weight")
     gb = None if grad_bias is None else _chk(grad_bias, "grad_bias", F32)
     _call("pda_linear_wgrad", x, _chk(x, "x", F32), _chk(grad_out, "grad_out", F32), _chk(grad_weight, "grad_weight", F32),
           gb, _chk(scratch, "scratch", torch.uint8), tokens, in_features, out_features)
@@ -411,6 +502,14 @@
     _numel_ok(x_gamma, in_features, "x_gamma"); _numel_ok(x_beta, in_features, "x_beta")
     nbytes = _wgrad_scratch_bytes(tokens, in_features, out_features)
     scratch = torch.empty((nbytes,), dtype=torch.uint8, device=x.device)
+    group = _open_group()
+    if group is not None:
+        slices = ctypes.c_int(0)
+        _call("pda_linear_wgrad_bn_partials", x, _chk(x, "x", F32), _chk(grad_out, "grad_out", F32), scratch.data_ptr(), tokens,
+              in_features, out_features, _chk(x_mean_invstd, "x_mean_invstd", F32), _chk(x_gamma, "x_gamma", F32),
+              _chk(x_beta, "x_beta", F32), ctypes.byref(slices))
+        group.add(_wgrad_entry(scratch, slices.value, grad_weight, None, in_features, out_features), scratch, grad_weight)
+        return 1
     _call("pda_linear_wgrad_bn", x, _chk(x, "x", F32), _chk(grad_out, "grad_out", F32), _chk(grad_weight, "grad_weight", F32), None,
           _chk(scratch, "scratch", torch.uint8), tokens, in_features, out_features, _chk(x_mean_invstd, "x_mean_invstd", F32),
           _chk(x_gamma, "x_gamma", F32), _chk(x_beta, "x_beta", F32))
diff --git a/pdanet_amd/pointnet2_utils.py b/pdanet_amd/pointnet2_utils.py
--- a/pdanet_amd/pointnet2_utils.py
+++ b/pdanet_amd/pointnet2_utils.py
@@ -1,5 +1,6 @@
 from typing import List, Tuple
 
+import functools
 import os
 
 import torch
@@ -489,6 +490,14 @@
     return list(DensityNetFusedMulti.apply(metas, *xs, *params))
 
 
+def _grouped_param_grads(backward):
+    @functools.wraps(backward)
+    def grouped(ctx, *grads):
+        with pointnet2.param_grad_group():
+            return backward(ctx, *grads)
+    return grouped
+
+
 class LinearLongTokens(Function):
     MIN_TOKENS = 4096
     SPLIT_MIN_TOKENS = 32768
@@ -802,6 +811,7 @@
         return y
 
     @staticmethod
+    @_grouped_param_grads
     def backward(ctx, dy):
         x, st1, src1_s, qkv, lse, a_s, ssum, st2, src2_s, h, h_s, n1w, in_w, out_w, n2w, w1, w2, arg = ctx.saved_tensors
         G, S, D = x.shape
@@ -845,7 +855,8 @@
         del dqkv, dqkv2
         d_x = torch.empty_like(x)
         gn1w, gn1b = torch.empty_like(n1w), torch.empty_like(n1w)
-        pointnet2.layer_norm_bwd(x, d_src1, n1w, st1, d_x, gn1w, gn1b, scratch, T, D)
+        scratch1 = torch.empty_like(scratch)
+        pointnet2.layer_norm_bwd(x, d_src1, n1w, st1, d_x, gn1w, gn1b, scratch1, T, D)
         return d_x, gn1w, gn1b, gwi, gbi, gwo, gbo, gn2w, gn2b, gw1, gb1, gw2, gb2, None, None, None, None
 
 
@@ -1207,6 +1218,7 @@
         return out
 
     @staticmethod
+    @_grouped_param_grads
     def backward(ctx, grad_out):
         xyz, new_xyz, feats_pm, idx, w1, w2, w3, g1, b1, g2, b2, g3, b3, z1, z2, z3, mi1, mi2, mi3, arg = ctx.saved_tensors
         B, M, ns = idx.shape
@@ -1254,7 +1266,11 @@
                 g_pts = torch.zeros((B, N, c1), dtype=torch.float32, device=dev)
                 pointnet2.group_rows_grad(B, N, c1, M * ns, gz1, idx, g_pts)
             g_pts = g_pts.view(B * N, c1)
-            dw1[:, 3:] = _wgrad(feats_pm.view(B * N, C), g_pts, torch.empty((c1, C), dtype=torch.float32, device=dev), False)[0]
+            x_pts = feats_pm.view(B * N, C)
+            if pointnet2.param_grad_group_open() and LINEAR_WGRAD_KERNEL and LinearLongTokens.kernel_wins(x_pts, dw1[:, 3:]):
+                pointnet2.linear_wgrad(x_pts, g_pts, dw1[:, 3:], None, B * N, C, c1)
+            else:
+                dw1[:, 3:] = _wgrad(x_pts, g_pts, torch.empty((c1, C), dtype=torch.float32, device=dev), False)[0]
             g_feats = _gemm_nn(g_pts, w1c[:, 3:].contiguous()).view(B, N, C) if ctx.needs_input_grad[2] else None
         return None, g_new, g_feats, None, dw1, dw2, dw3, dg1, db1, dg2, db2, dg3, db3, None
 
@@ -1442,6 +1458,7 @@
         return y
 
     @staticmethod
+    @_grouped_param_grads
     def backward(ctx, dy):
         x, st1, src1, qkv, lse, a, ssum, st2, src2, h, n1w, in_w, out_w, n2w, w1, w2, arg, cnt, off, rowmap = ctx.saved_tensors
         U, D = x.shape
@@ -1473,7 +1490,8 @@
         del dqkv
         d_x = torch.empty_like(x)
         gn1w, gn1b = torch.empty_like(n1w), torch.empty_like(n1w)
-        pointnet2.layer_norm_bwd(x, d_src1, n1w, st1, d_x, gn1w, gn1b, scratch, U, D)
+        scratch1 = torch.empty_like(scratch)
+        pointnet2.layer_norm_bwd(x, d_src1, n1w, st1, d_x, gn1w, gn1b, scratch1, U, D)
         return d_x, None, gn1w, gn1b, gwi, gbi, gwo, gbo, gn2w, gn2b, gw1, gb1, gw2, gb2, None, None, None
 
 
```
